# imazen/image-webp

Measured on AMD Instinct MI355X. Metric: 1920x1080 lossy encodes/s (Q75, method 4), higher is better.
Workload: dtype int32; 1 GPU; encode_frame_lossy 1920x1080 RGBA Q75 m4; device_batch=1024, distinct_frames=4, mbs_per_frame=8160, parallelism=frames sharded over 1 GPU(s), steps_pipelined=True, pipeline_lanes=2

## Files before the change

image-webp_amd/csrc/zw_enc_kernels.hip:

```cpp
#include "zw_dev.h"

#include <type_traits>

#include "zw_enc_rows.h"
#include "zw_enc_pairfinal.h"

#define ZW_PH_N 28

#ifdef ZW_NW
#define ZW_NW1 ZW_NW
#define ZW_NW2 ZW_NW
#endif
#ifndef ZW_NW1
#define ZW_NW1 12
#endif
#ifndef ZW_NW2
#define ZW_NW2 12
#endif
#define NW_MAX (ZW_NW1 > ZW_NW2 ? ZW_NW1 : ZW_NW2)
#ifndef ZW_DYN_PRIO
#define ZW_DYN_PRIO 1
#endif
#ifndef ZW_DYN_PRIO1
#define ZW_DYN_PRIO1 2
#endif
#ifndef ZW_P1_LUMA_MAX
#define ZW_P1_LUMA_MAX 3
#endif
#ifndef ZW_CHAIN_PRIO
#define ZW_CHAIN_PRIO 3
#endif
#ifndef ZW_LUMA_PRIO
#define ZW_LUMA_PRIO 0
#endif

template <int PASS> struct PassShape {
    static constexpr int NW = PASS == 1 ? ZW_NW1 : ZW_NW2;
    static constexpr int WG = NW * 64;
};

struct EncArgs {
    const uint8_t *Y, *U, *V;
    const uint8_t* alpha;
    const ZwFrameParams* params;
    const ZwLevelCosts* lcost;
    int8_t* derr;
    ZwMbOut* out;
    uint8_t *ry, *ru, *rv;
    size_t ysz, csz;
    int mbw, mbh, pass;
    int* dbg;
    uint8_t* rows;
    uint32_t* sizes;
    int nframes;
};

struct MbLds {
    uint8_t sy[256], su[64], sv[64];
    uint8_t ws[17 * ZW_BPS];
    uint8_t left_y[20], left_u[12], left_v[12], left_c[12];
    int8_t left_derr[4];
    uint8_t modes[16];
    int16_t lev[25][16];
};

struct WaveLds {
    MbLds mb;
    uint8_t cu[9 * ZW_BPS], cv[9 * ZW_BPS];
    uint32_t uvc[64][8];
    int dc[64];
    int y2d[64];
    int y2cost[4];
    int V[2][40];
    int nzt[4], nzl[4];
    int misc[16];
    uint32_t pst[2][4];
    uint8_t win_y[32], win_u[8], win_v[8], win_c[12];
    int8_t win_d[4];
#ifdef ZW_PHASE_PROF
    unsigned long long ph[ZW_PH_N];
#endif
};


struct Ctx {
    const EncArgs* a;
    const ZwFrameParams* P;
    int method;
    const ZwSegment* S;
    const ZwSegment* Sl;
    const LdsTables* T;
    WaveLds* W;
    MbLds* M;
    uint8_t *top_y, *top_u, *top_v, *top_c;
    int8_t* top_derr;
    const uint8_t *srcY, *srcU, *srcV;
    const uint8_t *sY, *sU, *sV;
    int ys, cs;
    int mbx, mby, lane, seg;
    int f;
    int oy, oc, ocx, od;
};

__device__ void build_luma_border(const Ctx& C, int part = 2)
{
    uint8_t* ws = C.M->ws;
    const int l = C.lane;
    const int mbw = C.a->mbw;
    const bool want = part == 2 || (part == 0 ? (l < 17 || l >= 32) : (l >= 17 && l < 32));
    if (!want) {
    } else if (l < 32) {
        int v;
        if (l == 0) v = C.mby == 0 ? 127 : (C.mbx == 0 ? 129 : C.M->left_y[0]);
        else if (C.mby == 0) v = 127;
        else if (l <= 16) v = C.top_y[C.oy + l - 1];
        else if (C.mbx == mbw - 1) v = C.top_y[C.oy + 15];
        else v = C.top_y[C.oy + l - 1];
        ws[l] = (uint8_t)v;
        if (l >= 17 && l < 21) {
            ws[4 * ZW_BPS + l] = (uint8_t)v;
            ws[8 * ZW_BPS + l] = (uint8_t)v;
            ws[12 * ZW_BPS + l] = (uint8_t)v;
        }
    } else if (l < 48) {
        int i = l - 32;
        ws[(i + 1) * ZW_BPS] = C.mbx == 0 ? 129 : C.M->left_y[1 + i];
    }
    wsync();
}

__device__ void build_chroma_border(const Ctx& C)
{
    const int l = C.lane;
    if (l < 34) {
        const int pl = l >= 17;
        const int i = pl ? l - 17 : l;
// ... 1641 lines not shown
            }
        }
#pragma unroll
        for (int k = 0; k < 8; k++)
            asm volatile("v_writelane_b32 %0, %1, %2" : "+v"(cf[0][0]) : "s"(__builtin_amdgcn_readfirstlane(dcs[k])), "i"(k));
    }
    int dq[2][4];
    int nz = 0;
#pragma unroll
    for (int c = 0; c < 2; c++)
#pragma unroll
        for (int r = 0; r < 4; r++) {
            const bool dcs = c == 0 && r == 0;
            const uint32_t iq = dcs ? (h ? S.uv.iq[1] : S.uv.iq[0]) : S.uv.iq[1];
            const uint32_t bias = dcs ? (h ? S.uv.bias[1] : S.uv.bias[0]) : S.uv.bias[1];
            const int q_ = dcs ? (int)(h ? S.uv.q[1] : S.uv.q[0]) : (int)S.uv.q[1];
            const int lv = quantz(cf[c][r], iq, bias);
            nz |= lv;
            if (act) C.M->lev[17 + b][izz_of(4 * r + 2 * h + c)] = (int16_t)lv;
            dq[c][r] = m24(lv, q_);
        }
    uint32_t r01[2], r32[2];
    idct_recon_pair(dq, p01, p32, h, r01, r32);
    if (act) {
        uint8_t* w = pl ? W->cv : W->cu;
#pragma unroll
        for (int r = 0; r < 2; r++) {
            uint8_t* row = w + (by * 4 + 2 * h + r + 1) * ZW_BPS + 1 + bx * 4;
            row[0] = (uint8_t)(r01[r] & 255u);
            row[1] = (uint8_t)(r01[r] >> 16);
            row[2] = (uint8_t)(r32[r] >> 16);
            row[3] = (uint8_t)(r32[r] & 255u);
        }
    }
    const int nzb = (nz | hx_partner(nz)) != 0;
    int any = 0;
#pragma unroll
    for (int k = 0; k < 8; k++) {
        uv_nz[k] = __builtin_amdgcn_readlane(nzb, k);
        any |= uv_nz[k];
    }
    wsync();
    return any;
}

__device__ void store_luma_borders(const Ctx& C)
{
    const int l = C.lane;
    if (l < 17) C.M->left_y[l] = C.M->ws[l * ZW_BPS + 16];
    else if (l < 33) C.top_y[C.oy + (l - 17)] = C.M->ws[16 * ZW_BPS + (l - 17) + 1];
    if (C.a->ry && l < 64) {
        uint8_t* ry = C.a->ry + (size_t)C.f * C.a->ysz + (size_t)C.mby * 16 * C.ys + C.mbx * 16;
        for (int k = l; k < 256; k += 64) ry[(size_t)(k >> 4) * C.ys + (k & 15)] = C.M->ws[((k >> 4) + 1) * ZW_BPS + 1 + (k & 15)];
    }
    wsync();
}
__device__ void store_chroma_borders(const Ctx& C)
{
    const int l = C.lane;
    WaveLds* W = C.W;
    if (l < 9) {
        C.M->left_u[l] = W->cu[l * ZW_BPS + 8];
        C.M->left_v[l] = W->cv[l * ZW_BPS + 8];
    } else if (l < 17) {
        C.top_u[C.oc + (l - 9)] = W->cu[8 * ZW_BPS + (l - 9) + 1];
        C.top_v[C.oc + (l - 9)] = W->cv[8 * ZW_BPS + (l - 9) + 1];
    }
    if (C.a->ru) {
        uint8_t* ru = C.a->ru + (size_t)C.f * C.a->csz + (size_t)C.mby * 8 * C.cs + C.mbx * 8;
        uint8_t* rv = C.a->rv + (size_t)C.f * C.a->csz + (size_t)C.mby * 8 * C.cs + C.mbx * 8;
        const int k = l;
        ru[(size_t)(k >> 3) * C.cs + (k & 7)] = W->cu[((k >> 3) + 1) * ZW_BPS + 1 + (k & 7)];
        rv[(size_t)(k >> 3) * C.cs + (k & 7)] = W->cv[((k >> 3) + 1) * ZW_BPS + 1 + (k & 7)];
    }
    wsync();
}

__device__ void write_levels(const Ctx& C, int first_blk, int nblk, bool zero)
{
    ZwMbOut* o = C.a->out + (size_t)C.f * C.a->mbw * C.a->mbh + (size_t)C.mby * C.a->mbw + C.mbx;
    uint32_t* dst = (uint32_t*)&o->levels[first_blk][0];
    const uint32_t* srcl = (const uint32_t*)&C.M->lev[first_blk][0];
    for (int k = C.lane; k < nblk * 8; k += 64) dst[k] = zero ? 0u : srcl[k];
}

struct UvQ {
    int pl;
    uint8_t* w;
    const uint8_t* sp;
    uint8_t* top;
    uint8_t* left;
};

DI void uvq_border(const Ctx& C, const UvQ& U)
{
    const int l = C.lane;
    if (l < 17) {
        if (l == 0) U.w[0] = C.mby == 0 ? 127 : (C.mbx == 0 ? 129 : U.left[0]);
        else if (l <= 8) U.w[l] = C.mby == 0 ? 127 : U.top[C.mbx * 8 + l - 1];
        else U.w[(l - 8) * ZW_BPS] = C.mbx == 0 ? 129 : U.left[l - 8];
    }
    wsync();
}

DI int uvq_rcost(const int av[4], int q, const LdsTables* T)
{
    unsigned nz = 0, big = 0;
    int part = 0;
#pragma unroll
    for (int r = 0; r < 4; r++) {
        const int n = 4 * r + q;
        nz |= (unsigned)min(av[r], 1) << n;
        big |= (unsigned)(av[r] >= 2) << n;
        part += T->lfc[min(av[r], 2047)];
    }
    nz = (unsigned)quad_or((int)nz);
    big = (unsigned)quad_or((int)big);
    const int sum = quad_sum(part);
    const int last = 31 - __clz((int)nz);
    const int ctx_t = ((big >> max(last, 0)) & 1u) ? 2 : 1;
    const int tail = (int)T->beob[2][band_of(min(last + 1, 15))][ctx_t] & -(int)(last < 15);
    const int head = (int)T->binit[2][0][0];
    return csel(last < 0, (int)T->beob[2][0][0], head + sum + tail);
}

DI int uvq_pick(const Ctx& C, const UvQ& U, int* xch, int* xflag, int seq)
{
    const ZwSegment& S = *C.S;
    const LdsTables* T = C.T;
    WaveLds* W = C.W;
    const int l = C.lane, m = l >> 4, b = (l >> 2) & 3, q = l & 3, bx = b & 1, by = b >> 1;
    const int above = C.mby != 0, left = C.mbx != 0;
    int dc;
    {
        const int i = l & 15;
        const int v = (int)U.w[csel(i < 8, (i + 1) * ZW_BPS, i - 7)] & -(int)(i < 8 ? left : above);
        const int su = __builtin_amdgcn_readlane(red16(v), 0);
        const int shf = 2 + left + above;
        dc = (above | left) ? (su + (1 << (shf - 1))) >> shf : 128;
    }
    uint32_t p01, p32, s01, s32;
    {
        const int cm = -(int)(m & 1), rm = -(int)(m >= 2);
        const int P = U.w[0];
        const int ro = csel(m == 0, dc, csel(m == 3, -P, 0));
        const uint8_t* tp = U.w + 1 + bx * 4;
        const uint32_t c01 = pack_lo(tp[0] & cm, tp[1] & cm), c32 = pack_lo(tp[3] & cm, tp[2] & cm);
        const int y = by * 4 + q;
        const int rv = (U.w[(y + 1) * ZW_BPS] & rm) + ro;
        const uint32_t rvv = pack_lo(rv, rv);
        p01 = clamp_pk(add_pk(c01, rvv));
        p32 = clamp_pk(add_pk(c32, rvv));
        const uint32_t sw = *(const uint32_t*)(U.sp + y * 8 + bx * 4);
        s01 = __builtin_amdgcn_perm(0u, sw, 0x0c010c00u);
        s32 = __builtin_amdgcn_perm(0u, sw, 0x0c020c03u);
    }
    const uint32_t R01 = sub_pk(s01, p01), R32 = sub_pk(s32, p32);
    int cf[4];
    uvq_fdct(add_pk(R01, R32), sub_pk(R01, R32), q, cf);
    {
        uint32_t* e = W->uvc[l];
        e[0] = pack_lo(cf[0], cf[1]);
        e[1] = pack_lo(cf[2], cf[3]);
        e[2] = p01;
        e[3] = p32;
    }
// ... 501 lines not shown
template <int PASS> DI void luma_issue_prio(const int* progress, int prevw, int mbx, int mby, int mbw)
{
#if ZW_DYN_PRIO > 0
    int slack = mbw;
    if (mby > 0) {
        const int v = __builtin_amdgcn_readfirstlane(
            __hip_atomic_load(&progress[prevw], __ATOMIC_RELAXED, __HIP_MEMORY_SCOPE_WORKGROUP));
        if ((v >> 16) == mby - 1) slack = (v & 0xffff) - mbx - 1;
    }
    constexpr int dp = PASS == 1 ? ZW_DYN_PRIO1 : ZW_DYN_PRIO;
    const int p = slack >= dp * 3 ? 3 : (slack >= dp * 2 ? 2 : (slack >= dp ? 1 : 0));
    set_prio(PASS == 1 ? min(p, ZW_P1_LUMA_MAX) : p);
#endif
}

DI uint32_t mb_luma(Ctx& C, int lm, bool i4reuse, uint32_t i4nz, bool trel)
{
    int ynz[16];
    uint32_t r = (uint32_t)(final_luma(C, lm, trel, ynz, i4reuse ? (int)i4nz : -1) != 0) << 16;
#pragma unroll
    for (int k = 0; k < 16; k++) r |= (uint32_t)(ynz[k] != 0) << k;
    return r;
}
DI uint32_t mb_chroma(Ctx& C, int cm)
{
    int uvnz[8];
    uint32_t r = (uint32_t)(final_chroma(C, cm, C.top_derr + C.od, uvnz) != 0) << 8;
#pragma unroll
    for (int k = 0; k < 8; k++) r |= (uint32_t)(uvnz[k] != 0) << k;
    return r;
}
template <int PASS> DI void mb_finish(Ctx& C, int lm, int cm, uint32_t lres, uint32_t cres, bool chroma_borders)
{
    const EncArgs& a = *C.a;
    const int lane = C.lane, mbw = a.mbw;
    const size_t nmb = (size_t)mbw * a.mbh;
    int ynz[16], uvnz[8];
#pragma unroll
    for (int k = 0; k < 16; k++) ynz[k] = (int)((lres >> k) & 1u);
#pragma unroll
    for (int k = 0; k < 8; k++) uvnz[k] = (int)((cres >> k) & 1u);
    const int lnz = (int)((lres >> 16) & 1u), cnz = (int)((cres >> 8) & 1u);
    ZwMbOut* o = a.out + (size_t)C.f * nmb + (size_t)C.mby * mbw + C.mbx;
    if (PASS == 2) {
        const int skip = !(lnz | cnz);
        if (lane == 0) {
            uint8_t* tc = C.top_c + C.ocx;
            uint8_t* lc = C.M->left_c;
            if (skip) {
                for (int k = 1; k < 9; k++) tc[k] = lc[k] = 0;
                if (lm != 4) tc[0] = lc[0] = 0;
            } else {
                if (lm != 4) {
                    int y2nz = 0;
                    for (int n = 0; n < 16; n++) y2nz |= C.M->lev[16][n] != 0;
                    tc[0] = lc[0] = (uint8_t)y2nz;
                }
                for (int x = 0; x < 4; x++) tc[1 + x] = (uint8_t)ynz[12 + x];
                for (int y = 0; y < 4; y++) lc[1 + y] = (uint8_t)ynz[y * 4 + 3];
                tc[5] = (uint8_t)uvnz[2];
                tc[6] = (uint8_t)uvnz[3];
                lc[5] = (uint8_t)uvnz[1];
                lc[6] = (uint8_t)uvnz[3];
                tc[7] = (uint8_t)uvnz[6];
                tc[8] = (uint8_t)uvnz[7];
                lc[7] = (uint8_t)uvnz[5];
                lc[8] = (uint8_t)uvnz[7];
            }
            o->skip = (uint8_t)skip;
            o->chroma_mode = (uint8_t)cm;
        }
        if (chroma_borders) store_chroma_borders(C);
        write_levels(C, 0, 25, skip);
        if (a.sizes) {
            int e = 0;
            if (lane < 25 && !skip) {
                const uint32_t* lw = (const uint32_t*)C.M->lev[lane];
#pragma unroll
                for (int q = 0; q < 8; q++) {
                    const uint32_t v = lw[q];
                    e = (v >> 16) ? 2 * q + 2 : ((v & 0xffffu) ? 2 * q + 1 : e);
                }
            }
            const int r16 = red16(e);
            const int es = __builtin_amdgcn_readlane(r16, 0) + __builtin_amdgcn_readlane(r16, 16);
            if (lane == 0)
                a.sizes[(size_t)C.f * nmb + (size_t)C.mby * mbw + C.mbx] = (uint32_t)(1 + (lm == 4 ? 8 : 0) + 25 + 2 * es);
        }
    } else {
        write_levels(C, 0, 17, false);
        if (lane == 0) o->skip = 0;
    }
    if (lane == 0) {
        o->luma_mode = (uint8_t)lm;
        o->segment = (uint8_t)C.seg;
    }
    if (lane < 16) o->bpred[lane] = lm == 4 ? C.M->modes[lane] : 0;
    store_luma_borders(C);
}
template <int PASS> DI void mb_store(Ctx& C, int lm, int cm, bool i4reuse, uint32_t i4nz, bool trel)
{
    [[maybe_unused]] const int lane = C.lane;
    PH_START();
    const uint32_t lres = mb_luma(C, lm, i4reuse, i4nz, trel);
    PH_MARK(4);
    const uint32_t cres = PASS == 2 ? mb_chroma(C, cm) : 0u;
    PH_MARK(5);
    mb_finish<PASS>(C, lm, cm, lres, cres, true);
}

template <int PASS> DI void chain_quad(const EncWg& G, Ctx& C)
{
    const EncArgs& a = *G.a;
    const int mbw = a.mbw, mbh = a.mbh, f = G.f, lane = C.lane;
    const size_t nmb = (size_t)mbw * mbh;
    if (lane < 4) C.M->left_derr[lane] = 0;
    const int pl = __builtin_amdgcn_readfirstlane(G.wv);
    UvQ U;
    U.pl = pl;
    U.w = G.W->cu;
    U.sp = C.M->su;
    U.top = pl ? G.top_v : G.top_u;
    U.left = C.M->left_u;
    const uint8_t* const P0 = (pl ? a.V : a.U) + (size_t)f * a.csz;
    const int cs = mbw * 8;
    auto fetch_uv = [&](int mbx, int mby) {
        MbFetch r;
        r.y = lane < 16 ? *(const uint32_t*)(P0 + (size_t)(mby * 8 + (lane >> 1)) * cs + mbx * 8 + (lane & 1) * 4) : 0u;
        r.c = 0;
        r.alpha = a.alpha[(size_t)f * nmb + (size_t)mby * mbw + mbx];
        return r;
    };
    C.ys = mbw * 16;
    C.cs = cs;
    MbFetch nx = fetch_uv(0, 0);
    int seq = 0;
    for (int mby = 0; mby < mbh; mby++) {
        if (lane < 12) C.M->left_u[lane] = 129;
        wsync();
        for (int mbx = 0; mbx < mbw; mbx++) {
            PH_START();
            const int lane = opaque_lane(threadIdx.x & 63);
            C.lane = lane;
            const MbFetch cur = nx;
            if (mbx + 1 < mbw) nx = fetch_uv(mbx + 1, mby);
            else if (mby + 1 < mbh) nx = fetch_uv(0, mby + 1);
            C.mbx = mbx;
            C.mby = mby;
            if (lane < 16) ((uint32_t*)C.M->su)[lane] = cur.y;
            wsync();
            const int seg = __builtin_amdgcn_readfirstlane((int)G.seg_lut[cur.alpha]);
            C.seg = seg;
            C.S = C.Sl + seg;
            uvq_border(C, U);
            const int cm = uvq_pick(C, U, G.xch, G.xflag, ++seq);
            PH_MARK(8);
            uvq_final(C, U, cm, G.top_derr + mbx * 4);
            PH_MARK(9);
            uvq_store_borders(C, U);
            ZwMbOut* o = a.out + (size_t)f * nmb + (size_t)mby * mbw + mbx;
            if (pl == 0 && lane == 0) o->chroma_mode = (uint8_t)cm;
            write_levels(C, 17 + 4 * pl, 4, false);
            wsync();
        }
    }
    for (int i = lane; i < mbw * 2; i += 64) {
        const int j = (i >> 1) * 4 + pl * 2 + (i & 1);
        a.derr[(size_t)f * mbw * 4 + j] = G.top_derr[j];
    }
}

template <int PASS, int FP> DI void chain_one(const EncWg& G, Ctx& C)
{
    const EncArgs& a = *G.a;
    const int mbw = a.mbw, mbh = a.mbh, lane = C.lane;
    const size_t nmb = (size_t)mbw * mbh;
    const int cfr = FP == 2 ? G.wv : 0;
    const bool has_chain = cfr < G.nf;
    const FrameLds F = frame_lds<PASS>(G, cfr);
    ctx_enter(C, F, &G.W->mb, 0, 0);
    if (lane < 4) C.M->left_derr[lane] = 0;
    MbFetch nx = fetch_mb(&a, F.f, lane, 0, 0);
    for (int mby = 0; has_chain && mby < mbh; mby++) {
        if (lane < 12) {
            C.M->left_u[lane] = 129;
            C.M->left_v[lane] = 129;
        }
        wsync();
        for (int mbx = 0; mbx < mbw; mbx++) {
            PH_START();
            const int lane = opaque_lane(threadIdx.x & 63);
            C.lane = lane;
            const MbFetch cur = nx;
            if (mbx + 1 < mbw) nx = fetch_mb(&a, F.f, lane, mbx + 1, mby);
            else if (mby + 1 < mbh) nx = fetch_mb(&a, F.f, lane, 0, mby + 1);
            setup_ctx(C, &a, F.seg_lut, G.W, mbx, mby, cur);
            C.oc = mbx * 8;
            C.ocx = mbx * 12;
            build_chroma_border(C);
            const int cm = pick_uv<PASS>(C);
            PH_MARK(8);
            int uvnz[8];
            final_chroma(C, cm, F.top_derr + mbx * 4, uvnz);
            PH_MARK(9);
            store_chroma_borders(C);
            ZwMbOut* o = a.out + (size_t)F.f * nmb + (size_t)mby * mbw + mbx;
            if (lane == 0) o->chroma_mode = (uint8_t)cm;
            write_levels(C, 17, 8, false);
            wsync();
        }
    }
    for (int i = lane; has_chain && i < mbw * 4; i += 64) a.derr[(size_t)F.f * mbw * 4 + i] = F.top_derr[i];
}

DI void ctx_pair(const Ctx& C, const FrameLds& F0, const FrameLds& F1, MbLds* const Mp[2], int mbx, int mby, int seg0,
                 int seg1, Ctx& CA, Ctx& CB)
{
    CA = CB = C;
    CA.lane = CB.lane = opaque_lane(threadIdx.x & 63);
    ctx_enter(CA, F0, Mp[0], mbx, mby);
    ctx_enter(CB, F1, Mp[1], mbx, mby);
    CA.seg = seg0;
    CB.seg = seg1;
    CA.S = CA.Sl + seg0;
    CB.S = CB.Sl + seg1;
}

template <int PASS, int NW, int NCW> DI void luma_pairs(const EncWg& G, Ctx& C)
{
    const EncArgs& a = *G.a;
    WaveLds* const W = G.W;
    int* const progress = G.progress;
    const int mbw = a.mbw, mbh = a.mbh, lane = C.lane;
    const int nf = __builtin_amdgcn_readfirstlane(G.nf), wv = __builtin_amdgcn_readfirstlane(G.wv);
    const FrameLds F[2] = {frame_lds<PASS>(G, 0), frame_lds<PASS>(G, 1)};
    MbLds* const Mp[2] = {&W->mb, G.M2};
    const int K = F[0].method <= 3 ? 3 : (F[0].method == 4 ? 4 : 10);
    const bool same_k = nf == 1 || (F[1].method == F[0].method && F[1].trel == F[0].trel);
    using RP = typename std::conditional<PASS == 1, PairRowSchedule1<NW, NCW>, RowSchedule<PASS, false, NW, NCW, true>>::type;
    for (int mby = RP::first_row(wv, mbh); mby < mbh; mby = RP::next_row(wv, mby, mbh)) {
#pragma unroll
        for (int fr = 0; fr < 2; fr++) row_start(Mp[fr], lane);
        wsync();
        const int prevw = __builtin_amdgcn_readfirstlane(mby > 0 ? RP::wave_of_row(mby - 1, mbh) : 0);
        auto wait_above = [&](int need) {
            if (mby > 0) wait_row(progress, prevw, (mby - 1) * 65536 + need);
        };
        for (int mbx = 0; mbx < mbw; mbx++) {
            PH_START();
            const int lane = opaque_lane(threadIdx.x & 63);
            C.lane = lane;
            auto enter = [&](int fr) {
                C.lane = opaque_lane(threadIdx.x & 63);
                ctx_enter(C, F[fr], Mp[fr], mbx, mby);
            };
            auto pst = [&](int fr, int k) { return (uint32_t)__builtin_amdgcn_readfirstlane((int)W->pst[fr][k]); };
            auto enter_seg = [&](int fr, uint32_t sm) {
                enter(fr);
                C.seg = (int)(sm >> 8);
                C.S = C.Sl + C.seg;
            };
            wait_above(min(mbx + 1, mbw));
            luma_issue_prio<PASS>(progress, prevw, mbx, mby, mbw);
            PH_MARK(0);
#pragma unroll
            for (int fr = 0; fr < 2; fr++) {
                if (fr >= nf) {
                    if (lane == 0) W->pst[fr][0] = 0;
                    continue;
                }
                enter(fr);
                const MbFetch fm = fetch_mb(&a, C.f, lane, mbx, mby);
                setup_ctx(C, &a, F[fr].seg_lut, W, mbx, mby, fm);
                build_luma_border(C, 0);
                int l_;
                unsigned long long s_;
                pick_i16<PASS>(C, l_, s_);
                const bool n_ = C.method > 1 && (C.method >= 5 || s_ > 211ull * C.S->l_mode || l_ != 0);
                if (lane == 0) {
                    W->pst[fr][0] = (uint32_t)l_ | ((uint32_t)n_ << 4) | ((uint32_t)C.seg << 8);
                    W->pst[fr][1] = (uint32_t)s_;
                    W->pst[fr][2] = (uint32_t)(s_ >> 32);
                    W->pst[fr][3] = 0;
                }
                wsync();
            }
            wsync();
            PH_MARK(1);
            const uint32_t s0 = pst(0, 0), s1 = pst(1, 0);
            const bool n0 = (s0 >> 4) & 1u, n1 = (s1 >> 4) & 1u;
            if (n0 || n1) wait_above(min(mbx + 2, mbw));
// ... 223 lines not shown
template <int PASS, bool ROWS, int FP = 1> DI void encode_body(const EncArgs& a)
{
    using SH = EncShape<PASS, ROWS, FP>;
    extern __shared__ __attribute__((aligned(16))) uint8_t smem[];
    const int lane = threadIdx.x & 63;
    const EncWg G = enc_carve<PASS, ROWS, FP>(a, smem);
    const bool chain_wg = PASS == 1 && (ROWS ? blockIdx.x == 0 : G.wv < SH::NCW);
    enc_fill<PASS, ROWS, FP>(G, chain_wg);

    Ctx C;
    C.a = &a;
    C.W = G.W;
    C.lane = lane;
    ctx_enter(C, frame_lds<PASS>(G, 0), &G.W->mb, 0, 0);
    ph_init(G, lane);

    if (chain_wg) {
        __builtin_amdgcn_s_setprio(ZW_CHAIN_PRIO);
        if constexpr (SH::NCH == 2 && !SH::PAIR) chain_quad<PASS>(G, C);
        else chain_one<PASS, FP>(G, C);
    }
    if (!chain_wg || SH::PAIR) {
        if (PASS == 1) __builtin_amdgcn_s_setprio(ZW_LUMA_PRIO);
        if constexpr (SH::PAIR) luma_pairs<PASS, SH::NW, SH::NCW>(G, C);
        else luma_rows<PASS, ROWS, SH::NW, SH::NCH>(G, C);
    }
    ph_flush<PASS>(G, lane);
}

extern "C" __global__ __launch_bounds__(PassShape<1>::WG) void k_encode_pass1(EncArgs a) { encode_body<1, false>(a); }
extern "C" __global__ __launch_bounds__(PassShape<1>::WG) void k_encode_pass1_fp(EncArgs a) { encode_body<1, false, 2>(a); }
extern "C" __global__ __launch_bounds__(PassShape<2>::WG) void k_encode_pass2(EncArgs a) { encode_body<2, false>(a); }
extern "C" __global__ __launch_bounds__(PassShape<2>::WG) void k_encode_pass2_fp(EncArgs a) { encode_body<2, false, 2>(a); }
extern "C" __global__ __launch_bounds__(64 * RowsShape<1>::NW) void k_encode_rows_pass1(EncArgs a) { encode_body<1, true>(a); }
extern "C" __global__ __launch_bounds__(64) void k_encode_rows_pass2(EncArgs a) { encode_body<2, true>(a); }

static size_t encode_lds_bytes(int mbw, int nw, bool rows, int pass, int fp = 1)
{
    return EncLds(mbw, rows, pass).bytes(nw, fp);
}

static bool encode_fp_for(int pass, int mbw, int nframes)
{
    static const int mode2 = [] { const char* e = getenv("ZW_ENC_FP"); return e && *e ? atoi(e) : -1; }();
    static const int mode1 = [] { const char* e = getenv("ZW_ENC_FP1"); return e && *e ? atoi(e) : mode2; }();
    const int mode = pass == 1 ? mode1 : mode2;
    static const int cus = [] {
        int dev = 0;
        hipDeviceProp_t prop;
        return hipGetDevice(&dev) == hipSuccess && hipGetDeviceProperties(&prop, dev) == hipSuccess &&
                       prop.multiProcessorCount > 0
                   ? prop.multiProcessorCount
                   : 256;
    }();
    if (mode == 0 || nframes < 2) return false;
    if (encode_lds_bytes(mbw, pass == 1 ? PassShape<1>::NW : PassShape<2>::NW, false, pass, 2) > 160 * 1024) return false;
    return mode == 1 || nframes >= 2 * cus;
}
extern "C" int zwk_encode_fp(int pass, int mbw, int nframes) { return encode_fp_for(pass, mbw, nframes) ? 1 : 0; }

extern "C" int zwk_encode_max_mbw(int rows)
{
    int lo = 1, hi = 65536 / 16;
    while (lo < hi) {
        const int mid = (lo + hi + 1) / 2;
        const bool ok = rows ? encode_lds_bytes(mid, RowsShape<1>::NW, true, 1) <= 160 * 1024 &&
                                   encode_lds_bytes(mid, RowsShape<2>::NW, true, 2) <= 160 * 1024
                             : encode_lds_bytes(mid, PassShape<1>::NW, false, 1) <= 160 * 1024 &&
                                   encode_lds_bytes(mid, PassShape<2>::NW, false, 2) <= 160 * 1024;
        if (ok) lo = mid;
        else hi = mid - 1;
    }
    return lo;
}

extern "C" size_t zwk_encode_rows_bytes(int mbw, int mbh, int nframes)
{
    return ZW_ROWS_HDR + (size_t)nframes * RowsLayout(mbw, mbh).frame;
}

extern "C" hipError_t zwk_encode(hipStream_t s, int pass, const uint8_t* Y, const uint8_t* U, const uint8_t* V,
                                 const uint8_t* alpha, const ZwFrameParams* params, const ZwLevelCosts* lcost,
                                 int8_t* derr, ZwMbOut* out, uint8_t* ry, uint8_t* ru, uint8_t* rv, size_t ysz,
                                 size_t csz, int mbw, int mbh, int nframes, int* dbg, uint8_t* rows, uint32_t* sizes)
{
    EncArgs a;
    a.dbg = dbg;
    a.sizes = pass == 2 ? sizes : nullptr;
    a.Y = Y; a.U = U; a.V = V; a.alpha = alpha; a.params = params; a.lcost = lcost; a.derr = derr; a.out = out;
    a.ry = ry; a.ru = ru; a.rv = rv; a.ysz = ysz; a.csz = csz; a.mbw = mbw; a.mbh = mbh; a.pass = pass;
    a.rows = rows;
    a.nframes = nframes;
    static const bool attr_set = []() {
        (void)hipFuncSetAttribute((const void*)k_encode_pass1, hipFuncAttributeMaxDynamicSharedMemorySize, 160 * 1024);
        (void)hipFuncSetAttribute((const void*)k_encode_pass2, hipFuncAttributeMaxDynamicSharedMemorySize, 160 * 1024);
        (void)hipFuncSetAttribute((const void*)k_encode_pass2_fp, hipFuncAttributeMaxDynamicSharedMemorySize, 160 * 1024);
        (void)hipFuncSetAttribute((const void*)k_encode_pass1_fp, hipFuncAttributeMaxDynamicSharedMemorySize, 160 * 1024);
        (void)hipFuncSetAttribute((const void*)k_encode_rows_pass1, hipFuncAttributeMaxDynamicSharedMemorySize, 160 * 1024);
        (void)hipFuncSetAttribute((const void*)k_encode_rows_pass2, hipFuncAttributeMaxDynamicSharedMemorySize, 160 * 1024);
        return true;
    }();
    (void)attr_set;
    if (rows) {
        if (pass == 1) {
            constexpr int nw = RowsShape<1>::NW;
            hipLaunchKernelGGL(k_encode_rows_pass1, dim3(1 + (mbh + nw - 1) / nw, nframes), dim3(64 * nw),
                               encode_lds_bytes(mbw, nw, true, 1), s, a);
        } else {
            hipLaunchKernelGGL(k_encode_rows_pass2, dim3(mbh, nframes), dim3(64), encode_lds_bytes(mbw, 1, true, 2), s,
                               a);
        }
        return hipGetLastError();
    }
    if (encode_fp_for(pass, mbw, nframes)) {
        if (pass == 1)
            hipLaunchKernelGGL(k_encode_pass1_fp, dim3((nframes + 1) / 2), dim3(PassShape<1>::WG),
                               encode_lds_bytes(mbw, PassShape<1>::NW, false, 1, 2), s, a);
        else
            hipLaunchKernelGGL(k_encode_pass2_fp, dim3((nframes + 1) / 2), dim3(PassShape<2>::WG),
                               encode_lds_bytes(mbw, PassShape<2>::NW, false, 2, 2), s, a);
        return hipGetLastError();
    }
    const size_t lds = encode_lds_bytes(mbw, pass == 1 ? PassShape<1>::NW : PassShape<2>::NW, false, pass);
    if (pass == 1) hipLaunchKernelGGL(k_encode_pass1, dim3(nframes), dim3(PassShape<1>::WG), lds, s, a);
    else hipLaunchKernelGGL(k_encode_pass2, dim3(nframes), dim3(PassShape<2>::WG), lds, s, a);
    return hipGetLastError();
}
```

image-webp_amd/csrc/zw_host.cpp:

```cpp
#include <hip/hip_runtime.h>
#include <immintrin.h>

#include <algorithm>
#include <chrono>
#include <atomic>
#include <sys/resource.h>
#include <sys/syscall.h>
#include <unistd.h>
#include <time.h>
#include <condition_variable>
#include <mutex>
#include <new>
#include <cstdio>
#include <cstdlib>
#include <cstring>
#include <deque>
#include <memory>
#include <thread>
#include <vector>

#include "../../include/zwebp.h"
#include "zw_common.h"
#include "zw_host_emit.h"
#include "zw_host_internal.h"
#include "zw_ingest.h"
#include "zw_progress.h"

extern "C" {
hipError_t zwk_rgb2yuv(hipStream_t s, const uint8_t* img, int w, int h, int bpp, int mbw, int mbh, uint8_t* Y,
                       uint8_t* U, uint8_t* V, size_t img_stride, size_t ysz, size_t csz, int nframes);
hipError_t zwk_rgb2yuv_dev(hipStream_t s, const void* data, int layout, int dtype, int channels, size_t frame_stride,
                           size_t plane_stride, size_t row_stride, const float* scale, const float* bias, int w, int h,
                           int mbw, int mbh, uint8_t* Y, uint8_t* U, uint8_t* V, size_t ysz, size_t csz, int nframes);
hipError_t zwk_analysis(hipStream_t s, const uint8_t* Y, const uint8_t* U, const uint8_t* V, int mbw, int mbh,
                        size_t ysz, size_t csz, uint8_t* alpha, uint32_t* histo, int nframes);
hipError_t zwk_segments(hipStream_t s, uint32_t* histo, const ZwFrameParams* tmpl, ZwFrameParams* params,
                        int nframes);
hipError_t zwk_stats(hipStream_t s, const ZwMbOut* mbs, int mbw, int mbh, void* scratch, void* out, int nframes);
size_t zw_stats_scratch_bytes(int nmb, int nframes);
hipError_t zwk_pack(hipStream_t s, const ZwMbOut* mbs, int nmb, int nframes, uint8_t* eobs, uint32_t* sizes,
                     unsigned long long* counter, unsigned long long* frame_info, uint8_t* out, int sizes_ready);
hipError_t zwk_fdct_quant(hipStream_t s, const void* src, const void* pred, size_t n, const ZwMatrix* m, int first,
                          void* levels, void* recon, int cus);
hipError_t zwk_xform_mb(hipStream_t s, const uint8_t* Y, const uint8_t* U, const uint8_t* V, int src_bpp, int w,
                        int h, size_t img_stride, const uint8_t* recs, const void* segs, int mbw, int mbh, int nframes,
                        int16_t* levels, uint8_t* RY, uint8_t* RU, uint8_t* RV, uint32_t* queue, int qp,
                        uint32_t* qerr, int variant);
size_t zwk_xform_mb_seg_bytes(void);
size_t zwk_xform_mb_queue_bytes(int mbw, int mbh, int nframes);
void zwk_xform_mb_pack_segs(const ZwMatrix* m, int n, void* out);
hipError_t zwk_quant_blocks(hipStream_t s, const int* coeffs, const uint8_t* ctx0s, const ZwLevelCosts* lcost,
                            const uint8_t* probs, const void* args, int* levels, int* dq);
hipError_t zwk_encode(hipStream_t s, int pass, const uint8_t* Y, const uint8_t* U, const uint8_t* V,
                      const uint8_t* alpha, const ZwFrameParams* params, const ZwLevelCosts* lcost, int8_t* derr,
                      ZwMbOut* out, uint8_t* ry, uint8_t* ru, uint8_t* rv, size_t ysz, size_t csz, int mbw, int mbh,
                      int nframes, int* dbg, uint8_t* rows, uint32_t* sizes = nullptr);
size_t zwk_encode_rows_bytes(int mbw, int mbh, int nframes);
int zwk_encode_max_mbw(int rows);
int zwk_encode_fp(int pass, int mbw, int nframes);
}

extern "C" const char* zw_strerror(int code)
{
    switch (code) {
    case ZW_OK: return "ok";
    case ZW_EINVALID_DIMENSIONS: return "invalid dimensions";
    case ZW_EINVALID_BUFFER_SIZE: return "invalid buffer size";
    case ZW_EINVAL: return "invalid argument";
    case ZW_EDEVICE: return "device error";
    case ZW_EUNSUPPORTED: return "unsupported";
    case ZW_ENOMEM: return "out of memory";
    case ZW_EVP8_MAGIC: return "invalid VP8 magic";
    case ZW_ECOLORSPACE: return "invalid VP8 color space";
    case ZW_ELUMA_MODE: return "invalid luma prediction mode";
    case ZW_EINTRA_MODE: return "invalid intra prediction mode";
    case ZW_ECHROMA_MODE: return "invalid chroma prediction mode";
    case ZW_EBITSTREAM: return "bitstream error";
    case ZW_EUNSUPPORTED_FEATURE: return "unsupported feature";
    case ZW_ENOT_ENOUGH_INIT_DATA: return "not enough VP8 init data";
    case ZW_ECHUNK_HEADER: return "invalid chunk header";
    case ZW_EWEBP_SIGNATURE: return "invalid WEBP signature";
    case ZW_ECHUNK_MISSING: return "an expected chunk was missing";
    case ZW_EINCONSISTENT_SIZES: return "inconsistent image sizes";
    case ZW_EIMAGE_TOO_LARGE: return "image too large";
    case ZW_EALPHA_PREPROCESSING: return "invalid alpha preprocessing";
    case ZW_ECOMPRESSION_METHOD: return "invalid compression method";
    case ZW_EHUFFMAN: return "invalid lossless Huffman code";
    case ZW_ETRANSFORM: return "invalid lossless transform";
    case ZW_ECOLOR_CACHE_BITS: return "invalid color cache bits";
    case ZW_ELOSSLESS_SIGNATURE: return "invalid lossless signature";
    case ZW_EVERSION_NUMBER: return "invalid lossless version number";
    default: return "unknown error";
    }
}

static std::atomic<int> g_ctx_alive{0};
bool zw_ctx_any_alive() { return g_ctx_alive.load(std::memory_order_acquire) > 0; }

extern "C" int zw_ctx_create(int device, zw_ctx** out)
{
    if (!out) return ZW_EINVAL;
    *out = nullptr;
    int n = 0;
    if (hipGetDeviceCount(&n) != hipSuccess || n <= 0 || device < 0 || device >= n) return ZW_EDEVICE;
    HIPOK(hipSetDevice(device));
    zw_ctx* c = new zw_ctx();
    c->device = device;
    g_ctx_alive.fetch_add(1, std::memory_order_acq_rel);
    *out = c;
    return ZW_OK;
}

struct AgentFind {
    uint32_t bdf, domain;
    hsa_agent_t gpu{}, cpu{};
    bool gpu_ok = false, cpu_ok = false;
};
static hsa_status_t find_agents_cb(hsa_agent_t a, void* data)
{
    AgentFind* F = (AgentFind*)data;
    hsa_device_type_t t;
    if (hsa_agent_get_info(a, HSA_AGENT_INFO_DEVICE, &t) != HSA_STATUS_SUCCESS) return HSA_STATUS_SUCCESS;
    if (t == HSA_DEVICE_TYPE_CPU && !F->cpu_ok) {
        F->cpu = a;
        F->cpu_ok = true;
    } else if (t == HSA_DEVICE_TYPE_GPU) {
        uint32_t bdf = 0, dom = 0;
        (void)hsa_agent_get_info(a, (hsa_agent_info_t)HSA_AMD_AGENT_INFO_BDFID, &bdf);
        (void)hsa_agent_get_info(a, (hsa_agent_info_t)HSA_AMD_AGENT_INFO_DOMAIN, &dom);
        if (bdf == F->bdf && dom == F->domain) {
            F->gpu = a;
            F->gpu_ok = true;
        }
    }
    return HSA_STATUS_SUCCESS;
}

static int sdma_probe_locked(zw_ctx* c)
{
// ... 276 lines not shown
    size_t n = 0;
    bool alloc(size_t count)
    {
        free();
        if (hipHostMalloc((void**)&p, count * sizeof(T) + 64, hipHostMallocDefault) != hipSuccess) {
            p = nullptr;
            return false;
        }
        n = count;
        memset((void*)p, 0, count * sizeof(T));
        return true;
    }
    void free()
    {
        pinned_free(p);
        p = nullptr;
        n = 0;
    }
    T* data() { return p; }
    T& operator[](size_t i) { return p[i]; }
    const T& operator[](size_t i) const { return p[i]; }
    size_t size() const { return n; }
    ~Pinned() { free(); }
};

struct FetchBuf {
    uint8_t* pack = nullptr;
    size_t cap = 0;
    Pinned<unsigned long long> finfo;
    Pinned<unsigned long long> total;
    void release()
    {
        pinned_free(pack);
        pack = nullptr;
        cap = 0;
    }
};

enum LaneEvent { EV_YUV_BEGIN, EV_YUV_END, EV_P1_BEGIN, EV_P1_END, EV_P2_BEGIN, EV_P2_END, EV_STATS_QUEUED, EV_COUNT };
enum KernelMs { KMS_RGB2YUV, KMS_ANALYSIS, KMS_PASS1, KMS_PASS2, KMS_COUNT };
enum HostMs { HMS_FETCH, HMS_STATS, HMS_FETCH2, HMS_EMIT, HMS_COUNT };
enum { PIPE_MS_HOST = KMS_COUNT, PIPE_MS_EMIT_CPU = KMS_COUNT + HMS_COUNT, PIPE_MS_COUNT };

struct PipeLane {
    int f0 = 0, n = 0;
    int chunk = 0;
    hipStream_t stream = nullptr;
    std::vector<hipEvent_t> cev;
    static int pass_slot(int c, int pass) { return 2 * c + pass - 1; }
    hipEvent_t pass_done(int c, int pass) const { return cev[pass_slot(c, pass)]; }
    hipEvent_t ev[EV_COUNT] = {};
    unsigned long long* d_ctr = nullptr;
    uint8_t* d_rows = nullptr;
    FetchBuf fb[3];
    Pinned<ZwStatsOut> h_stats;
    float kms[KMS_COUNT] = {0, 0, 0, 0};
    double hms[HMS_COUNT] = {0, 0, 0, 0};
    double emit_cpu_ms = 0;
    bool pair2 = false;
    int p2_frames = 0;
    bool pair1 = false;
    int p1_frames = 0;
    int rc = 0;
    std::vector<hipStream_t> ustreams;
    std::vector<hipEvent_t> uev[2], rev[2];
    std::vector<uint8_t*> ustage;
    std::vector<hsa_signal_t> usig;
};

struct zw_pipe {
    zw_ctx* ctx;
    int n, w, h, color, bpp, quality, method, mbw, mbh, nmb, qi, filter;
    size_t img_stride, ysz, csz;
    uint8_t *d_img = nullptr, *d_Y = nullptr, *d_U = nullptr, *d_V = nullptr;
    uint8_t *d_ry = nullptr, *d_ru = nullptr, *d_rv = nullptr, *d_alpha = nullptr;
    uint32_t* d_histo = nullptr;
    ZwFrameParams *d_tmpl = nullptr, *d_params = nullptr;
    ZwLevelCosts* d_lcost = nullptr;
    int8_t* d_derr = nullptr;
    ZwMbOut *d_out1 = nullptr, *d_out2 = nullptr;
    int* d_dbg = nullptr;
    ZwStatsOut* d_stats = nullptr;
    void* d_stats_tmp = nullptr;
    bool host_stats = false;
    uint8_t* d_eobs = nullptr;
    uint32_t* d_sizes = nullptr;
    unsigned long long *d_finfo = nullptr, *d_finfo2 = nullptr;
    uint8_t *d_pack = nullptr, *d_pack2 = nullptr;
    size_t pack_stride = 0;
    Pinned<ZwFrameParams> h_params;
    Pinned<ZwLevelCosts> h_lcost;
    std::vector<uint8_t> h_have_upd;
    std::vector<uint8_t> h_upd;
    int out_par = 0;
    std::vector<std::vector<uint8_t>> bitstreams;
    bool container = false;
    std::vector<const uint8_t*> host_frames;
    int nparts = 1;
    std::vector<PipeLane> lanes;
    std::vector<Progress> p1_stats;
    float kms[PIPE_MS_COUNT] = {0, 0, 0, 0, 0, 0, 0, 0, 0};
    bool trace = false;
    double trace_t0 = 0;
    std::mutex ews_mu;
    std::vector<std::unique_ptr<zwh::EmitWs>> ews;
    bool broken = false;
    uint8_t* d_img2 = nullptr;
    const uint8_t* const* host_src = nullptr;
    bool up_pack = false;
    uint8_t* img_buf(int parity) const { return parity ? d_img2 : d_img; }
    zw_device_images dev_in = {};
};

static void pipe_free(zw_pipe* p)
{
    if (!p) return;
    if (p->ctx && p->ctx->poisoned.load(std::memory_order_acquire)) p->d_img = p->d_img2 = nullptr;
    void* ptrs[] = {p->d_img, p->d_img2, p->d_Y, p->d_U, p->d_V, p->d_ry, p->d_ru, p->d_rv, p->d_alpha, p->d_histo,
                    p->d_tmpl, p->d_params, p->d_lcost, p->d_derr, p->d_out1, p->d_out2, p->d_dbg,
                    p->d_eobs, p->d_sizes, p->d_finfo, p->d_pack, p->d_finfo2, p->d_pack2, p->d_stats, p->d_stats_tmp};
    for (void* q : ptrs)
        if (q) (void)hipFree(q);
    for (PipeLane& L : p->lanes) {
        if (L.d_ctr) (void)hipFree(L.d_ctr);
        if (L.d_rows) (void)hipFree(L.d_rows);
        for (FetchBuf& b : L.fb) b.release();
        for (hipEvent_t e : L.ev)
            if (e) (void)hipEventDestroy(e);
        for (hipEvent_t e : L.cev)
            if (e) (void)hipEventDestroy(e);
        if (L.stream) (void)hipStreamDestroy(L.stream);
        for (hipStream_t u : L.ustreams) (void)hipStreamDestroy(u);
        for (uint8_t* b : L.ustage) pinned_free(b);
        if (!g_dma_poisoned.load())
            for (hsa_signal_t sg : L.usig) (void)hsa_signal_destroy(sg);
        for (int k = 0; k < 2; k++) {
            for (hipEvent_t e : L.uev[k])
                if (e) (void)hipEventDestroy(e);
            for (hipEvent_t e : L.rev[k])
                if (e) (void)hipEventDestroy(e);
        }
    }
    delete p;
}

static int pipe_lanes_for(int n, int device, int mbw)
{
    const char* e = getenv("ZW_PIPE_LANES");
    int g;
    if (e && *e) {
        g = atoi(e);
    } else {
        const int cus = device_cus(device);
        const bool fp = zwk_encode_fp(2, mbw, 2 * cus) != 0;
        g = n >= (fp ? 4 : 2) * cus ? 2 : 1;
    }
    if (g < 1) g = 1;
    if (g > 16) g = 16;
    while (g > 1 && n / g < 8) g--;
    return g;
}
static int pipe_chunk_for(int lane_frames, int device)
{
    const char* e = getenv("ZW_PIPE_CHUNK");
    int c = e ? atoi(e) : 0;
    if (c < 1) c = device_cus(device);
    return c > lane_frames ? lane_frames : c;
}
static bool pipe_rows_for(int chunk, int mbw, int mbh, int device)
{
    static const int batch_max_mbw = zwk_encode_max_mbw(0);
    if (mbw > batch_max_mbw) return true;
    const char* e = getenv("ZW_ENC_ROWS");
    if (e && *e) return atoi(e) != 0;
    return (long long)chunk * (mbh + 1) <= 12LL * device_cus(device);
}

extern "C" int zw_pipe_create(zw_ctx* ctx, int n, uint32_t width, uint32_t height, int color, uint8_t quality,
                              uint8_t method, zw_pipe** out)
{
    if (!ctx || !out || n <= 0) return ZW_EINVAL;
    *out = nullptr;
    if (!encode_dims_ok(width, height)) return ZW_EINVALID_DIMENSIONS;
    if (color < 0 || color > 3) return ZW_EINVAL;
    if (quality > 100) return ZW_EINVAL;
    HIPOK(hipSetDevice(ctx->device));
    zw_pipe* p = new zw_pipe();
    p->ctx = ctx;
    p->n = n;
    p->w = (int)width;
    p->h = (int)height;
    p->color = color;
    static const int bpp_of[4] = {1, 2, 3, 4};
    p->bpp = bpp_of[color];
    p->quality = quality;
    p->method = method > 6 ? 6 : method;
    p->mbw = (p->w + 15) / 16;
    p->mbh = (p->h + 15) / 16;
    p->nmb = p->mbw * p->mbh;
    p->img_stride = (size_t)p->w * p->h * p->bpp;
    p->ysz = (size_t)p->mbw * 16 * p->mbh * 16;
    p->csz = (size_t)p->mbw * 8 * p->mbh * 8;
    p->qi = zwh::quality_to_qi(quality);
    p->filter = zwh::filter_level_for(p->qi);
    p->pack_stride = (size_t)p->nmb * (1 + 8 + 25 + 800);
    const size_t N = (size_t)n;
    bool ok = hipMalloc(&p->d_img, N * p->img_stride + 64) == hipSuccess &&
              hipMalloc(&p->d_Y, N * p->ysz) == hipSuccess && hipMalloc(&p->d_U, N * p->csz) == hipSuccess &&
              hipMalloc(&p->d_V, N * p->csz) == hipSuccess && hipMalloc(&p->d_ry, N * p->ysz) == hipSuccess &&
              hipMalloc(&p->d_ru, N * p->csz) == hipSuccess && hipMalloc(&p->d_rv, N * p->csz) == hipSuccess &&
              hipMalloc(&p->d_alpha, N * p->nmb) == hipSuccess &&
              hipMalloc(&p->d_histo, N * 256 * sizeof(uint32_t)) == hipSuccess &&
              hipMalloc(&p->d_tmpl, sizeof(ZwFrameParams)) == hipSuccess &&
              hipMalloc(&p->d_params, N * sizeof(ZwFrameParams)) == hipSuccess &&
              hipMalloc(&p->d_lcost, N * sizeof(ZwLevelCosts)) == hipSuccess &&
              hipMalloc(&p->d_derr, N * p->mbw * 4) == hipSuccess &&
              hipMalloc(&p->d_out1, N * p->nmb * sizeof(ZwMbOut)) == hipSuccess &&
              hipMalloc(&p->d_out2, N * p->nmb * sizeof(ZwMbOut)) == hipSuccess &&
              hipMalloc(&p->d_eobs, N * p->nmb * 25) == hipSuccess &&
              hipMalloc(&p->d_sizes, N * p->nmb * sizeof(uint32_t)) == hipSuccess &&
              hipMalloc(&p->d_finfo, N * 2 * sizeof(unsigned long long)) == hipSuccess &&
              hipMalloc(&p->d_pack, N * p->pack_stride) == hipSuccess &&
              hipMalloc(&p->d_finfo2, N * 2 * sizeof(unsigned long long)) == hipSuccess &&
              hipMalloc(&p->d_pack2, N * p->pack_stride) == hipSuccess;
    ok = ok && hipMemset(p->d_histo, 0, N * 256 * sizeof(uint32_t)) == hipSuccess;
    p->host_stats = getenv("ZW_HOST_STATS") != nullptr;
    ok = ok && (p->host_stats || (hipMalloc(&p->d_stats, N * sizeof(ZwStatsOut)) == hipSuccess &&
                                  hipMalloc(&p->d_stats_tmp, zw_stats_scratch_bytes(p->nmb, n)) == hipSuccess));
    const int G = pipe_lanes_for(n, ctx->device, p->mbw);
    p->lanes.resize(G);
    for (int g = 0; ok && g < G; g++) {
        PipeLane& L = p->lanes[g];
        L.f0 = (int)((long long)n * g / G);
        L.n = (int)((long long)n * (g + 1) / G) - L.f0;
        L.chunk = pipe_chunk_for(L.n, ctx->device);
        for (FetchBuf& b : L.fb) ok = ok && b.finfo.alloc(2 * (size_t)L.chunk) && b.total.alloc(1);
        ok = ok && (p->host_stats || L.h_stats.alloc((size_t)L.n));
        const int nch = (L.n + L.chunk - 1) / L.chunk;
        L.cev.assign(2 * (size_t)nch, nullptr);
        ok = ok && hipStreamCreateWithFlags(&L.stream, hipStreamNonBlocking) == hipSuccess &&
             hipMalloc(&L.d_ctr, 2 * (size_t)nch * ZW_PACK_CTR_WORDS * sizeof(unsigned long long)) == hipSuccess &&
             hipMemset(L.d_ctr, 0, 2 * (size_t)nch * ZW_PACK_CTR_WORDS * sizeof(unsigned long long)) == hipSuccess;
        if (ok && pipe_rows_for(L.chunk, p->mbw, p->mbh, ctx->device)) {
            const size_t rb = zwk_encode_rows_bytes(p->mbw, p->mbh, L.chunk);
            ok = hipMalloc(&L.d_rows, rb) == hipSuccess && hipMemset(L.d_rows, 0, rb) == hipSuccess;
            if (ok && getenv("ZW_ENC_FORCE_ERROR")) ok = hipMemset(L.d_rows, 1, 1) == hipSuccess;
        }
        L.pair2 = ok && !L.d_rows && nch >= 2 && zwk_encode_fp(2, p->mbw, 2 * L.chunk);
        L.pair1 = ok && !L.d_rows && nch >= 2 && zwk_encode_fp(1, p->mbw, 2 * L.chunk);
        for (int i = 0; ok && i < EV_COUNT; i++) ok = hipEventCreate(&L.ev[i]) == hipSuccess;
        for (size_t i = 0; ok && i < L.cev.size(); i++)
            ok = hipEventCreateWithFlags(&L.cev[i], hipEventDisableTiming) == hipSuccess;
    }
    if (!ok) {
        pipe_free(p);
        return ZW_ENOMEM;
    }
    if (!p->h_params.alloc(2 * N) || !p->h_lcost.alloc(N)) {
        pipe_free(p);
        return ZW_ENOMEM;
    }
    p->h_have_upd.assign(2 * N, 0);
    p->h_upd.assign(2 * N * 4 * 8 * 3 * 11, 0);
    p->bitstreams.resize(N);
    ZwFrameParams t;
    memset(&t, 0, sizeof t);
    t.width = p->w;
    t.height = p->h;
    t.mbw = p->mbw;
    t.mbh = p->mbh;
    t.method = p->method;
    t.do_trellis = p->method >= 4;
    t.base_qi = p->qi;
    t.filter_level = p->filter;
    t.skip_prob = 200;
    memcpy(t.probs, zwh::COEFF_PROBS, sizeof t.probs);
    if (hipMemcpy(p->d_tmpl, &t, sizeof t, hipMemcpyHostToDevice) != hipSuccess) {
        pipe_free(p);
        return ZW_EDEVICE;
    }
    *out = p;
    return ZW_OK;
}

extern "C" void zw_pipe_destroy(zw_pipe* p)
{
    if (p) (void)hipSetDevice(p->ctx->device);
    pipe_free(p);
}

extern "C" void* zw_pipe_input_device_ptr(zw_pipe* p) { return p ? p->d_img : nullptr; }

extern "C" int zw_pipe_set_container(zw_pipe* p, int enable, const uint8_t* const* host_frames)
{
    if (!p) return ZW_EINVAL;
    if (!enable) {
        p->container = false;
        p->host_frames.clear();
        return ZW_OK;
    }
    const bool has_alpha = p->color == ZW_COLOR_LA8 || p->color == ZW_COLOR_RGBA8;
    if (has_alpha && p->dev_in.data) return ZW_EINVAL;
    if (has_alpha) {
        if (p->w > 16384 || p->h > 16384) return ZW_EINVALID_DIMENSIONS;
        if (!host_frames) return ZW_EINVAL;
        for (int i = 0; i < p->n; i++)
            if (!host_frames[i]) return ZW_EINVAL;
        p->host_frames.assign(host_frames, host_frames + p->n);
    }
    p->container = true;
    return ZW_OK;
// ... 12 lines not shown
        in->capacity < need)
        return ZW_EINVAL;
    const size_t es = (size_t)ing_elsize(in->dtype);
    if (!ing_madd(0, in->capacity, es, &bytes) || ((uintptr_t)in->data & (es - 1))) return ZW_EINVAL;
    HIPOK(hipSetDevice(ctx->device));
    hipPointerAttribute_t at;
    memset(&at, 0, sizeof at);
    if (hipPointerGetAttributes(&at, in->data) != hipSuccess) {
        (void)hipGetLastError();
        return ZW_EINVAL;
    }
    if (at.type != hipMemoryTypeDevice || at.device != ctx->device) return ZW_EINVAL;
    return ZW_OK;
}

extern "C" int zw_pipe_set_input_device(zw_pipe* p, const zw_device_images* in)
{
    if (!p) return ZW_EINVAL;
    if (!in) {
        p->dev_in = zw_device_images{};
        return ZW_OK;
    }
    if (const int r = check_device_input(p->ctx, in, p->n, (uint32_t)p->w, (uint32_t)p->h)) return r;
    if (!((p->color == ZW_COLOR_RGB8 && in->channels == 3) || (p->color == ZW_COLOR_RGBA8 && in->channels == 4)))
        return ZW_EINVAL;
    if (p->container && in->channels == 4) return ZW_EINVAL;
    p->dev_in = *in;
    return ZW_OK;
}

extern "C" int zw_pipe_set_token_partitions(zw_pipe* p, int nparts)
{
    if (!p || (nparts != 1 && nparts != 2 && nparts != 4 && nparts != 8)) return ZW_EINVAL;
    p->nparts = nparts;
    return ZW_OK;
}

extern "C" int zw_pipe_upload(zw_pipe* p, int frame, const uint8_t* data, size_t len)
{
    if (!p || frame < 0 || frame >= p->n || !data) return ZW_EINVAL;
    if (len != p->img_stride) return ZW_EINVALID_BUFFER_SIZE;
    HIPOK(hipMemcpy(p->d_img + (size_t)frame * p->img_stride, data, len, hipMemcpyHostToDevice));
    return ZW_OK;
}

static double now_ms()
{
    return std::chrono::duration<double, std::milli>(std::chrono::steady_clock::now().time_since_epoch()).count();
}
static long long thread_cpu_ns()
{
    timespec ts;
    clock_gettime(CLOCK_THREAD_CPUTIME_ID, &ts);
    return (long long)ts.tv_sec * 1000000000LL + ts.tv_nsec;
}

static hipError_t rows_reset(zw_pipe* p, PipeLane& L, int n)
{
    if (!L.d_rows) return hipSuccess;
    const size_t hdr = zwk_encode_rows_bytes(p->mbw, p->mbh, 0);
    return hipMemsetAsync(L.d_rows + hdr, 0, zwk_encode_rows_bytes(p->mbw, p->mbh, n) - hdr, L.stream);
}
static int rows_check(zw_pipe* p, PipeLane& L)
{
    if (!L.d_rows) return ZW_OK;
    int err = 0;
    HIPOK(hipMemcpy(&err, L.d_rows, sizeof err, hipMemcpyDeviceToHost));
    return err ? ZW_EDEVICE : ZW_OK;
}

static int chunk_pass1_encode(zw_pipe* p, PipeLane& L, int fa, int na, bool timed, bool write_recon = false)
{
    hipStream_t s = L.stream;
    const size_t F = (size_t)fa;
    if (timed) {
        HIPOK(hipEventRecord(L.ev[EV_P1_BEGIN], s));
        L.p1_frames = na;
    }
    HIPOK(rows_reset(p, L, na));
    HIPOK(zwk_encode(s, 1, p->d_Y + F * p->ysz, p->d_U + F * p->csz, p->d_V + F * p->csz, p->d_alpha + F * p->nmb,
                     p->d_params + F, nullptr, p->d_derr + F * p->mbw * 4, p->d_out1 + F * p->nmb,
                     write_recon ? p->d_ry + F * p->ysz : nullptr, write_recon ? p->d_ru + F * p->csz : nullptr,
                     write_recon ? p->d_rv + F * p->csz : nullptr, p->ysz, p->csz, p->mbw, p->mbh, na, nullptr,
                     L.d_rows));
    if (timed) HIPOK(hipEventRecord(L.ev[EV_P1_END], s));
    return ZW_OK;
}

static int chunk_prepass(zw_pipe* p, PipeLane& L, int fa, int na, bool timed, int parity, hipEvent_t uploaded,
                         hipEvent_t read)
{
    hipStream_t s = L.stream;
    const size_t F = (size_t)fa;
    const int n = na;
    if (uploaded) HIPOK(hipStreamWaitEvent(s, uploaded, 0));
    if (timed) HIPOK(hipEventRecord(L.ev[EV_YUV_BEGIN], s));
    const bool packed = uploaded && p->up_pack;
    if (const zw_device_images& D = p->dev_in; D.data) {
        const uint8_t* src = (const uint8_t*)D.data + F * D.frame_stride * (size_t)ing_elsize(D.dtype);
        HIPOK(zwk_rgb2yuv_dev(s, src, D.layout, D.dtype, D.channels, D.frame_stride, D.plane_stride, D.row_stride,
                              D.scale, D.bias, p->w, p->h, p->mbw, p->mbh, p->d_Y + F * p->ysz, p->d_U + F * p->csz,
                              p->d_V + F * p->csz, p->ysz, p->csz, n));
    } else {
        HIPOK(zwk_rgb2yuv(s, p->img_buf(parity) + F * p->img_stride, p->w, p->h, packed ? 3 : p->bpp, p->mbw, p->mbh,
                          p->d_Y + F * p->ysz, p->d_U + F * p->csz, p->d_V + F * p->csz, p->img_stride, p->ysz,
                          p->csz, n));
    }
    if (read) HIPOK(hipEventRecord(read, s));
    if (timed) HIPOK(hipEventRecord(L.ev[EV_YUV_END], s));
    HIPOK(zwk_analysis(s, p->d_Y + F * p->ysz, p->d_U + F * p->csz, p->d_V + F * p->csz, p->mbw, p->mbh, p->ysz,
                       p->csz, p->d_alpha + F * p->nmb, p->d_histo + F * 256, n));
    HIPOK(zwk_segments(s, p->d_histo + F * 256, p->d_tmpl, p->d_params + F, n));
    return ZW_OK;
}

static bool pass2_sizes(const zw_pipe* p) { return p->d_sizes != nullptr; }

static int chunk_pack(zw_pipe* p, PipeLane& L, int fa, int na, const ZwMbOut* d_out, int slot)
{
    const size_t F = (size_t)fa;
    const bool p2 = slot & 1;
    HIPOK(zwk_pack(L.stream, d_out + F * p->nmb, p->nmb, na, p->d_eobs + F * p->nmb * 25, p->d_sizes + F * p->nmb,
                   L.d_ctr + ZW_PACK_CTR_WORDS * slot, (p2 ? p->d_finfo2 : p->d_finfo) + 2 * F,
                   (p2 ? p->d_pack2 : p->d_pack) + F * p->pack_stride, p2 && pass2_sizes(p)));
    return ZW_OK;
}

static int chunk_fetch(zw_pipe* p, PipeLane& L, FetchBuf& B, int fa, int na, int slot, hipEvent_t ready)
{
    const size_t F = (size_t)fa;
    HIPOK(hipEventSynchronize(ready));
    int r = ctx_d2h(p->ctx, B.total.data(), L.d_ctr + ZW_PACK_CTR_WORDS * slot + 2, sizeof(unsigned long long));
    const bool p2 = slot & 1;
    if (!r)
        r = ctx_d2h(p->ctx, B.finfo.data(), (p2 ? p->d_finfo2 : p->d_finfo) + 2 * F,
                    2 * (size_t)na * sizeof(unsigned long long));
    if (r) return r;
    const unsigned long long total = B.total[0];
    if (total > B.cap) {
        B.release();
        const size_t cap = (size_t)(total * 1.25) + 4096;
        if (hipHostMalloc((void**)&B.pack, cap, hipHostMallocDefault) != hipSuccess) return ZW_ENOMEM;
        B.cap = cap;
    }
    return ctx_d2h(p->ctx, B.pack, (p2 ? p->d_pack2 : p->d_pack) + F * p->pack_stride, total);
}

static int chunk_fetch_stats(zw_pipe* p, PipeLane& L, int fa, int na, hipEvent_t ready)
{
    HIPOK(hipEventSynchronize(ready));
    return ctx_d2h(p->ctx, L.h_stats.data() + (fa - L.f0), p->d_stats + fa, (size_t)na * sizeof(ZwStatsOut));
}

static inline size_t hidx(const zw_pipe* p, int par, size_t f) { return (size_t)par * p->n + f; }

static int chunk_stats(zw_pipe* p, PipeLane& L, int fa, int na, int par)
{
    hipStream_t s = L.stream;
    const size_t F = (size_t)fa, n = (size_t)na;
    ZwFrameParams* hp = p->h_params.data() + hidx(p, par, F);
    {
        const int r = ctx_d2h(p->ctx, hp, p->d_params + F, n * sizeof(ZwFrameParams));
        if (r) return r;
    }
    parallel_for(na, [&](int i) {
        const size_t f = F + i, hf = hidx(p, par, f);
        zwh::Stats st;
        int sp;
        if (p->host_stats) {
            sp = zwh::replay_stats(st, L.fb[0].pack + L.fb[0].finfo[2 * i], p->mbw, p->mbh);
        } else {
            const ZwStatsOut& so = L.h_stats[f - L.f0];
            memcpy(st.s, so.s, sizeof st.s);
            sp = zwh::skip_prob(so.total_mbs, so.nonzero_mbs);
        }
        uint8_t* upd = p->h_upd.data() + hf * 4 * 8 * 3 * 11;
        bool have = zwh::updated_probs(st, (uint8_t(*)[8][3][11])upd);
        p->h_have_upd[hf] = have;
        ZwFrameParams& P = p->h_params[hf];
        P.skip_prob = sp;
        memcpy(P.probs, upd, sizeof P.probs);
        zwh::level_costs(p->h_lcost[f], (const uint8_t(*)[8][3][11])upd);
    });
    HIPOK(hipMemcpyAsync(p->d_params + F, hp, n * sizeof(ZwFrameParams), hipMemcpyHostToDevice, s));
    HIPOK(hipMemcpyAsync(p->d_lcost + F, p->h_lcost.data() + F, n * sizeof(ZwLevelCosts), hipMemcpyHostToDevice, s));
    return ZW_OK;
}

static int chunk_pass2(zw_pipe* p, PipeLane& L, int fa, int na, bool timed)
{
    hipStream_t s = L.stream;
    const size_t F = (size_t)fa;
    if (timed) {
        HIPOK(hipEventRecord(L.ev[EV_P2_BEGIN], s));
        L.p2_frames = na;
    }
    HIPOK(rows_reset(p, L, na));
    HIPOK(zwk_encode(s, 2, p->d_Y + F * p->ysz, p->d_U + F * p->csz, p->d_V + F * p->csz, p->d_alpha + F * p->nmb,
                     p->d_params + F, p->d_lcost + F, p->d_derr + F * p->mbw * 4, p->d_out2 + F * p->nmb,
                     p->d_ry + F * p->ysz, p->d_ru + F * p->csz, p->d_rv + F * p->csz, p->ysz, p->csz, p->mbw, p->mbh,
                     na, p->d_dbg ? p->d_dbg + F * p->nmb * 16 * 34 : nullptr, L.d_rows,
                     pass2_sizes(p) ? p->d_sizes + F * p->nmb : nullptr));
    if (timed) HIPOK(hipEventRecord(L.ev[EV_P2_END], s));
    return ZW_OK;
}

static void dump_emit_input(zw_pipe* p, const uint8_t* rec, size_t bytes, size_t hf)
{
    static const char* path = getenv("ZW_DUMP_EMIT");
    static std::atomic<int> done{0};
    if (!path || done.exchange(1)) return;
    FILE* fp = fopen(path, "wb");
    if (!fp) return;
    const uint32_t hdr[4] = {0x4d45575au, (uint32_t)sizeof(ZwFrameParams), (uint32_t)p->w, (uint32_t)p->h};
    const uint8_t have = p->h_have_upd[hf];
    const unsigned long long n = bytes;
    bool ok = fwrite(hdr, sizeof hdr, 1, fp) == 1 && fwrite(&p->h_params[hf], sizeof(ZwFrameParams), 1, fp) == 1 &&
              fwrite(&have, 1, 1, fp) == 1 && fwrite(p->h_upd.data() + hf * 4 * 8 * 3 * 11, 4 * 8 * 3 * 11, 1, fp) == 1 &&
              fwrite(&n, sizeof n, 1, fp) == 1 && fwrite(rec, 1, bytes, fp) == bytes;
    (void)ok;
    fclose(fp);
}

struct EmitWsLease {
    zw_pipe* p;
    std::atomic<long long>& to;
    const long long c0 = thread_cpu_ns();
    std::unique_ptr<zwh::EmitWs> ws;
    EmitWsLease(zw_pipe* p_, std::atomic<long long>& to_) : p(p_), to(to_)
    {
        {
            std::lock_guard<std::mutex> lk(p->ews_mu);
            if (!p->ews.empty()) {
                ws = std::move(p->ews.back());
                p->ews.pop_back();
            }
        }
        if (!ws) ws.reset(new (std::nothrow) zwh::EmitWs);
    }
    ~EmitWsLease()
    {
        if (!ws) return;
        {
            std::lock_guard<std::mutex> lk(p->ews_mu);
            p->ews.push_back(std::move(ws));
        }
        to.fetch_add(thread_cpu_ns() - c0, std::memory_order_relaxed);
    }
};

static int emit_task(zw_pipe* p, const FetchBuf& B, int fa, int par, int i0, int K, zwh::EmitWs* ws)
{
    const size_t F = (size_t)fa;
    const bool has_alpha = p->color == ZW_COLOR_LA8 || p->color == ZW_COLOR_RGBA8;
    std::vector<uint8_t>* vp8 = ws->out;
    std::vector<uint8_t>& alph = ws->alph;
    std::vector<uint8_t>* outs[zwh::EmitWs::kMax];
    for (int k = 0; k < K; k++) {
        const size_t f = F + i0 + k;
        outs[k] = p->container ? &vp8[k] : &p->bitstreams[f];
        outs[k]->clear();
    }
    const ZwFrameParams* Pk[zwh::EmitWs::kMax];
    const uint8_t* rk[zwh::EmitWs::kMax];
    bool hk[zwh::EmitWs::kMax];
    const uint8_t(*uk[zwh::EmitWs::kMax])[8][3][11];
    for (int k = 0; k < K; k++) {
        const size_t hf = hidx(p, par, F + i0 + k);
        Pk[k] = &p->h_params[hf];
        rk[k] = B.pack + B.finfo[2 * (i0 + k)];
        hk[k] = p->h_have_upd[hf] != 0;
        uk[k] = (const uint8_t(*)[8][3][11])(p->h_upd.data() + hf * 4 * 8 * 3 * 11);
    }
    try {
        zwh::emit_frames(outs, Pk, rk, K, p->nparts, p->w, p->h, hk, uk, ws);
    } catch (const std::bad_alloc&) {
        return ZW_ENOMEM;
    }
    if (!p->container) return ZW_OK;
    for (int k = 0; k < K; k++) {
        const size_t f = F + i0 + k;
        std::vector<uint8_t>& out = p->bitstreams[f];
        alph.clear();
        out.clear();
        if (has_alpha) {
// ... 69 lines not shown
        : p(p_), L(L_), emit(emit_), nb(nb_), nch((L_.n + L_.chunk - 1) / L_.chunk), host(p_->host_src != nullptr),
          G((int)p_->lanes.size()), lane_id((int)(&L_ - p_->lanes.data())), p1_order(G > 1 && emit_),
          uploaded(host ? L_.ustreams.size() : 0)
    {
    }
    ~LaneRun()
    {
        join_emitter();
        join_uploaders();
        if (p1_order) p->p1_stats[lane_id].stop();
    }

    int first(int c) const { return L.f0 + c * L.chunk; }
    int count(int c) const { return std::min(L.chunk, L.n - c * L.chunk); }
    template <class F>
    int for_launch_groups(bool paired, F fn) const
    {
        for (int c = 0; c < nch; c++) {
            const int c1 = (paired && (c & 1) == 0 && c + 1 < nch) ? c + 1 : c;
            if (const int r = fn(LaunchGroup{c, c1, first(c), first(c1) + count(c1) - first(c)})) return r;
            c = c1;
        }
        return ZW_OK;
    }
    int join_emitter()
    {
        if (em.joinable()) em.join();
        return emit_rc;
    }
    void join_uploaders()
    {
        if (up.empty()) return;
        if (p1_count < (long long)nb * nch) p1_queued.stop();
        for (auto& t : up) t.join();
        up.clear();
    }

    int p1_order_wait(int b)
    {
        if (!p1_order) return ZW_OK;
        const int prev = (lane_id + G - 1) % G;
        const long long need = lane_id == 0 ? b : b + 1;
        if (need <= 0 || !p->p1_stats[prev].wait_for(need)) return ZW_OK;
        HIPOK(hipStreamWaitEvent(L.stream, p->lanes[prev].ev[EV_STATS_QUEUED], 0));
        return ZW_OK;
    }
    int wait_uploaded(int b, int k)
    {
        for (Progress& u : uploaded)
            if (!u.wait_for((long long)b * nch + k + 1)) return ZW_EDEVICE;
        for (size_t u = 1; u < L.ustreams.size(); u++)
            HIPOK(hipStreamWaitEvent(L.stream, L.uev[b & 1][u * nch + k], 0));
        return ZW_OK;
    }
    int launch_pass1(int b, const LaunchGroup& g)
    {
        if (g.c0 == 0)
            if (const int r = p1_order_wait(b)) return r;
        return chunk_pass1_encode(p, L, g.fa, g.na, g.c0 == 0);
    }
    int queue_pass1_group(int b, const LaunchGroup& g)
    {
        const bool paired = g.c1 != g.c0;
        int r = ZW_OK;
        for (int k = g.c0; k <= g.c1 && !r; k++) {
            if (host && (r = wait_uploaded(b, k))) return r;
            r = chunk_prepass(p, L, first(k), count(k), k == 0, host ? (b & 1) : 0, host ? L.uev[b & 1][k] : nullptr,
                              host ? L.rev[b & 1][k] : nullptr);
            if (!r && !paired) r = launch_pass1(b, g);
            if (host && r) p1_queued.stop();
            if (host && !r) {
                p1_count++;
                p1_queued.advance();
            }
        }
        if (!r && paired) r = launch_pass1(b, g);
        for (int k = g.c0; k <= g.c1 && !r; k++) {
            if (p->host_stats) {
                r = chunk_pack(p, L, first(k), count(k), p->d_out1, PipeLane::pass_slot(k, 1));
            } else {
                const size_t F = (size_t)first(k);
                HIPOK(zwk_stats(L.stream, p->d_out1 + F * p->nmb, p->mbw, p->mbh,
                                (uint8_t*)p->d_stats_tmp + zw_stats_scratch_bytes(p->nmb, (int)F), p->d_stats + F,
                                count(k)));
            }
            if (!r) HIPOK(hipEventRecord(L.pass_done(k, 1), L.stream));
        }
        return r;
    }
    int queue_pass1(int b)
    {
        if (const int r = for_launch_groups(L.pair1, [&](const LaunchGroup& g) { return queue_pass1_group(b, g); }))
            return r;
        if (p1_order) {
            HIPOK(hipEventRecord(L.ev[EV_STATS_QUEUED], L.stream));
            p->p1_stats[lane_id].advance();
        }
        return ZW_OK;
    }
    int stats_and_pass2_group(int b, const LaunchGroup& g)
    {
        int r;
        for (int k = g.c0; k <= g.c1; k++) {
            const double t0 = now_ms();
            r = p->host_stats ? chunk_fetch(p, L, L.fb[0], first(k), count(k), PipeLane::pass_slot(k, 1),
                                            L.pass_done(k, 1))
                              : chunk_fetch_stats(p, L, first(k), count(k), L.pass_done(k, 1));
            if (r) return r;
            const double t1 = now_ms();
            if ((r = chunk_stats(p, L, first(k), count(k), b & 1))) return r;
            ms[HMS_STATS] += now_ms() - t1;
            ms[HMS_FETCH] += t1 - t0;
            if (p->trace)
                fprintf(stderr, "  lane %d batch %d chunk %d: p1 fetched %.1f stats done %.1f\n", L.f0, b, k,
                        t1 - p->trace_t0, now_ms() - p->trace_t0);
            if (emit && b > 0 && !fetched.wait_for((long long)(b - 1) * nch + k + 1)) {
                const int re = join_emitter();
                return re ? re : ZW_EDEVICE;
            }
        }
        r = chunk_pass2(p, L, g.fa, g.na, g.c0 == 0);
        for (int k = g.c0; k <= g.c1 && !r; k++) {
            if (emit) r = chunk_pack(p, L, first(k), count(k), p->d_out2, PipeLane::pass_slot(k, 2));
            if (!r && hipEventRecord(L.pass_done(k, 2), L.stream) != hipSuccess) r = ZW_EDEVICE;
        }
        return r;
    }
    int stats_and_pass2(int b)
    {
        return for_launch_groups(L.pair2, [&](const LaunchGroup& g) { return stats_and_pass2_group(b, g); });
    }
    int run()
    {
        for (int u = 0; u < (int)uploaded.size(); u++) up.emplace_back([this, u] { upload_chunks(u); });
        int r = queue_pass1(0);
        for (int b = 0; b < nb && !r; b++) {
            r = stats_and_pass2(b);
            if (!r && b + 1 < nb) r = queue_pass1(b + 1);
            if (!r && emit && !(r = join_emitter())) em = std::thread([this, b] { emit_thread(b); });
        }
        if (r) return r;
        if ((r = join_emitter())) return r;
        join_uploaders();
        if (up_rc.load()) return up_rc.load();
        p->out_par = (nb - 1) & 1;
        HIPOK(hipStreamSynchronize(L.stream));
        if ((r = rows_check(p, L))) return r;
        for (int i = 0; i < HMS_COUNT; i++) L.hms[i] = ms[i] / nb;
        L.emit_cpu_ms = 1e-6 * (double)emit_cpu.load() / nb;
        lane_times(L);
        return ZW_OK;
    }

    int upload_chunk_dma(int u, int b, int c)
    {
        const int U = (int)L.ustreams.size();
        uint8_t* dst = p->img_buf(b & 1) + (size_t)first(c) * p->img_stride;
        int r = ZW_OK;
        if (b >= 2 && hipEventSynchronize(L.rev[b & 1][c]) != hipSuccess) r = ZW_EDEVICE;
        bool busy[2] = {false, false};
        int k = 0;
        for (int i = u; i < count(c) && !r; i += U, k++) {
            const int sl = k & 1;
            if (busy[sl] && (r = sdma_wait(p->ctx, L.usig[2 * u + sl]))) break;
            const uint8_t* src = p->host_src[(size_t)b * p->n + first(c) + i];
            size_t bytes = p->img_stride;
            if (p->up_pack) {
// ... 223 lines not shown
                L.usig.push_back(sg);
            }
        }
        for (int k = 0; k < 2; k++) {
            while ((int)L.uev[k].size() < U * nch) {
                hipEvent_t a = nullptr;
                HIPOK(hipEventCreateWithFlags(&a, hipEventDisableTiming));
                L.uev[k].push_back(a);
            }
            while ((int)L.rev[k].size() < nch) {
                hipEvent_t a = nullptr;
                HIPOK(hipEventCreateWithFlags(&a, hipEventDisableTiming));
                L.rev[k].push_back(a);
            }
        }
    }
    {
        const char* pe = getenv("ZW_UPLOAD_PACK");
        p->up_pack = p->bpp == 4 && !p->lanes.empty() && !p->lanes[0].ustage.empty() && !(pe && atoi(pe) == 0);
    }
    p->host_src = frames;
    const int r = pipe_encode(p, nb);
    p->host_src = nullptr;
    p->up_pack = false;
    return r;
}

extern "C" int zw_pipe_encode_repeat(zw_pipe* p, int n) { return pipe_encode(p, n); }

extern "C" int zw_pipe_launch_frames(zw_pipe* p) { return p && !p->lanes.empty() ? p->lanes[0].chunk : 0; }

extern "C" int zw_pipe_lanes(zw_pipe* p) { return p ? (int)p->lanes.size() : 0; }

extern "C" int zw_pipe_kernel_times(zw_pipe* p, float* ms, int n)
{
    if (!p || !ms) return ZW_EINVAL;
    for (int i = 0; i < n && i < PIPE_MS_COUNT; i++) ms[i] = p->kms[i];
    return ZW_OK;
}

extern "C" int zw_pipe_output(zw_pipe* p, int frame, zw_bytes* out)
{
    if (!p || !out || frame < 0 || frame >= p->n) return ZW_EINVAL;
    const std::vector<uint8_t>& b = p->bitstreams[frame];
    out->data = (uint8_t*)malloc(b.size() ? b.size() : 1);
    if (!out->data) return ZW_ENOMEM;
    memcpy(out->data, b.data(), b.size());
    out->len = b.size();
    return ZW_OK;
}

extern "C" int zw_pipe_read_planes(zw_pipe* p, int frame, int which, uint8_t* y, uint8_t* u, uint8_t* v)
{
    if (!p || frame < 0 || frame >= p->n) return ZW_EINVAL;
    HIPOK(hipSetDevice(p->ctx->device));
    uint8_t* Y = which ? p->d_ry : p->d_Y;
    uint8_t* U = which ? p->d_ru : p->d_U;
    uint8_t* V = which ? p->d_rv : p->d_V;
    if (y) HIPOK(hipMemcpy(y, Y + (size_t)frame * p->ysz, p->ysz, hipMemcpyDeviceToHost));
    if (u) HIPOK(hipMemcpy(u, U + (size_t)frame * p->csz, p->csz, hipMemcpyDeviceToHost));
    if (v) HIPOK(hipMemcpy(v, V + (size_t)frame * p->csz, p->csz, hipMemcpyDeviceToHost));
    return ZW_OK;
}

extern "C" int zw_pipe_read_mbinfo(zw_pipe* p, int frame, int pass, uint8_t* modes, int16_t* levels)
{
    if (!p || frame < 0 || frame >= p->n) return ZW_EINVAL;
    HIPOK(hipSetDevice(p->ctx->device));
    std::vector<ZwMbOut> tmp(p->nmb);
    HIPOK(hipMemcpy(tmp.data(), (pass == 1 ? p->d_out1 : p->d_out2) + (size_t)frame * p->nmb,
                    p->nmb * sizeof(ZwMbOut), hipMemcpyDeviceToHost));
    for (int i = 0; i < p->nmb; i++) {
        if (modes) {
            uint8_t* m = modes + (size_t)i * 20;
            m[0] = tmp[i].luma_mode;
            m[1] = tmp[i].chroma_mode;
            m[2] = tmp[i].skip;
            m[3] = tmp[i].segment;
            memcpy(m + 4, tmp[i].bpred, 16);
        }
        if (levels) memcpy(levels + (size_t)i * 400, tmp[i].levels, 800);
    }
    return ZW_OK;
}

extern "C" int zw_pipe_read_probs(zw_pipe* p, int frame, uint8_t* probs, int* skip_prob)
{
    if (!p || frame < 0 || frame >= p->n) return ZW_EINVAL;
    const ZwFrameParams& P = p->h_params[hidx(p, p->out_par, (size_t)frame)];
    if (probs) memcpy(probs, P.probs, sizeof P.probs);
    if (skip_prob) *skip_prob = P.skip_prob;
    return ZW_OK;
}

extern "C" int zw_pipe_read_segments(zw_pipe* p, int frame, int32_t* seg_qi)
{
    if (!p || frame < 0 || frame >= p->n || !seg_qi) return ZW_EINVAL;
    const ZwFrameParams& P = p->h_params[hidx(p, p->out_par, (size_t)frame)];
    for (int i = 0; i < 4; i++) seg_qi[i] = P.seg[i].quant_index;
    return ZW_OK;
}

extern "C" int zw_pipe_enable_debug(zw_pipe* p)
{
    if (!p) return ZW_EINVAL;
    if (p->d_dbg) return ZW_OK;
    HIPOK(hipSetDevice(p->ctx->device));
    const size_t b = (size_t)p->n * p->nmb * 16 * 34 * sizeof(int);
    if (hipMalloc(&p->d_dbg, b) != hipSuccess) return ZW_ENOMEM;
    HIPOK(hipMemset(p->d_dbg, 0, b));
    return ZW_OK;
}

extern "C" int zw_pipe_read_debug(zw_pipe* p, int frame, int32_t* out)
{
    if (!p || !p->d_dbg || frame < 0 || frame >= p->n || !out) return ZW_EINVAL;
    HIPOK(hipSetDevice(p->ctx->device));
    const size_t b = (size_t)p->nmb * 16 * 34 * sizeof(int);
    HIPOK(hipMemcpy(out, (uint8_t*)p->d_dbg + (size_t)frame * b, b, hipMemcpyDeviceToHost));
    return ZW_OK;
}

extern "C" int zw_pipe_read_alpha(zw_pipe* p, int frame, uint8_t* alpha)
{
    if (!p || frame < 0 || frame >= p->n || !alpha) return ZW_EINVAL;
    HIPOK(hipSetDevice(p->ctx->device));
    HIPOK(hipMemcpy(alpha, p->d_alpha + (size_t)frame * p->nmb, p->nmb, hipMemcpyDeviceToHost));
    return ZW_OK;
}

static int check_encode_args(const uint8_t* data, size_t len, uint32_t width, uint32_t height, int color,
                             uint8_t quality)
{
    if (!encode_dims_ok(width, height)) return ZW_EINVALID_DIMENSIONS;
    if (color < 0 || color > 3) return ZW_EINVAL;
    static const int bpp_of[4] = {1, 2, 3, 4};
    if ((uint64_t)width * height * bpp_of[color] != len || !data) return ZW_EINVALID_BUFFER_SIZE;
    if (quality > 100) return ZW_EINVAL;
    return ZW_OK;
}

extern "C" int zw_encode_batch(zw_ctx* ctx, int n, const zw_image* imgs, uint8_t quality, uint8_t method,
                               zw_bytes* outs)
{
    return zw_encode_batch_ex(ctx, n, imgs, quality, method, 1, outs);
}

extern "C" int zw_encode_batch_ex(zw_ctx* ctx, int n, const zw_image* imgs, uint8_t quality, uint8_t method,
                                  int token_partitions, zw_bytes* outs)
{
    if (!ctx || n <= 0 || !imgs || !outs) return ZW_EINVAL;
    if (token_partitions != 1 && token_partitions != 2 && token_partitions != 4 && token_partitions != 8)
        return ZW_EINVAL;
    for (int i = 0; i < n; i++) {
        outs[i].data = nullptr;
        outs[i].len = 0;
        int r = check_encode_args(imgs[i].data, imgs[i].len, imgs[i].width, imgs[i].height, imgs[i].color, quality);
        if (r) return r;
        if (imgs[i].width != imgs[0].width || imgs[i].height != imgs[0].height || imgs[i].color != imgs[0].color)
            return ZW_EINVAL;
    }
    zw_pipe* p = nullptr;
    int r;
    const int key[5] = {(int)imgs[0].width, (int)imgs[0].height, imgs[0].color, quality, method};
    const bool one = n == 1;
    if (one) {
// ... 647 lines not shown
```

image-webp_amd/csrc/zw_pack_kernels.hip:

```cpp
#include "zw_dev.h"

#ifndef PK_WAVES
#define PK_WAVES 4
#endif

__device__ __forceinline__ int pk_mb_size(int luma, int eobsum) { return 1 + (luma == 4 ? 8 : 0) + 25 + 2 * eobsum; }

__device__ __forceinline__ int pk_word_eob(uint32_t v, int j)
{
    const int n0 = 2 * (j & 7);
    return (v >> 16) ? n0 + 2 : ((v & 0xffffu) ? n0 + 1 : 0);
}
__device__ __forceinline__ int max8(int e)
{
    e = max(e, __builtin_amdgcn_mov_dpp(e, 0xB1, 0xf, 0xf, false));
    e = max(e, __builtin_amdgcn_mov_dpp(e, 0x4E, 0xf, 0xf, false));
    e = max(e, __builtin_amdgcn_mov_dpp(e, 0x141, 0xf, 0xf, false));
    return e;
}

extern "C" __global__ __launch_bounds__(64 * PK_WAVES) void k_pack_size(const ZwMbOut* __restrict__ mbs, int nmb,
                                                                      int nframes, uint8_t* __restrict__ eobs,
                                                                      uint32_t* __restrict__ sizes)
{
    const size_t mb = (size_t)blockIdx.x * PK_WAVES + (threadIdx.x >> 6);
    const int lane = threadIdx.x & 63;
    if (mb >= (size_t)nmb * nframes) return;
    const ZwMbOut& M = mbs[mb];
    const uint32_t* W = (const uint32_t*)&M.levels[0][0];
    uint32_t w[4];
#pragma unroll
    for (int r = 0; r < 4; r++) w[r] = lane + 64 * r < 200 ? W[lane + 64 * r] : 0u;
    const int skip = M.skip;
    int s = 0;
#pragma unroll
    for (int r = 0; r < 4; r++) {
        const int j = lane + 64 * r;
        const int eob = skip ? 0 : max8(pk_word_eob(w[r], j));
        if ((j & 7) == 0 && j < 200) {
            eobs[mb * 25 + (j >> 3)] = (uint8_t)eob;
            s += eob;
        }
    }
#pragma unroll
    for (int o = 32; o >= 1; o >>= 1) s += __shfl_xor(s, o);
    if (lane == 0) sizes[mb] = (uint32_t)pk_mb_size(M.luma_mode, s);
}

extern "C" __global__ __launch_bounds__(1024) void k_pack_scan(uint32_t* __restrict__ sizes, int nmb,
                                                              unsigned long long* __restrict__ counter,
                                                              unsigned long long* __restrict__ frame_info)
{
    __shared__ uint32_t part[1024];
    __shared__ unsigned long long base;
    const int f = blockIdx.x, t = threadIdx.x;
    uint32_t* S = sizes + (size_t)f * nmb;
    const int per = (nmb + 1023) / 1024;
    const int b0 = t * per, b1 = min(b0 + per, nmb);
    uint32_t acc = 0;
    for (int i = b0; i < b1; i++) acc += S[i];
    part[t] = acc;
    __syncthreads();
    for (int o = 1; o < 1024; o <<= 1) {
        const uint32_t v = t >= o ? part[t - o] : 0;
        __syncthreads();
        part[t] += v;
        __syncthreads();
    }
    uint32_t run = part[t] - acc;
    for (int i = b0; i < b1; i++) {
        const uint32_t v = S[i];
        S[i] = run;
        run += v;
    }
    if (t == 1023) {
        const unsigned long long tot = part[1023];
        base = atomicAdd(counter, tot);
        frame_info[2 * f] = base;
        frame_info[2 * f + 1] = tot;
        __threadfence();
        if (atomicAdd(counter + 1, 1ull) == (unsigned long long)gridDim.x - 1) {
            __threadfence();
            const unsigned long long all = atomicAdd(counter, 0ull);
            counter[2] = all;
            atomicExch(counter, 0ull);
            atomicExch(counter + 1, 0ull);
        }
    }
}

extern "C" __global__ __launch_bounds__(64 * PK_WAVES) void k_pack_write(
    const ZwMbOut* __restrict__ mbs, int nmb, int nframes, const uint8_t* __restrict__ eobs,
    const uint32_t* __restrict__ offs, const unsigned long long* __restrict__ frame_info, uint8_t* __restrict__ out)
{
    const size_t mb = (size_t)blockIdx.x * PK_WAVES + (threadIdx.x >> 6);
    const int lane = threadIdx.x & 63;
    if (mb >= (size_t)nmb * nframes) return;
    const int f = (int)(mb / nmb);
    const ZwMbOut& M = mbs[mb];
    const uint32_t* W = (const uint32_t*)&M.levels[0][0];
    uint32_t w[4];
#pragma unroll
    for (int r = 0; r < 4; r++) w[r] = lane + 64 * r < 200 ? W[lane + 64 * r] : 0u;
    const uint32_t hw = *(const uint32_t*)&M;
    const uint32_t bp = lane < 8 ? *(const uint16_t*)&M.bpred[2 * lane] : 0u;
    uint8_t* o = out + frame_info[2 * f] + offs[mb];
    const int luma = (int)(hw & 255u), chroma = (int)((hw >> 8) & 255u), skip = (int)((hw >> 16) & 255u),
              seg = (int)(hw >> 24);
    const int hdr = 1 + (luma == 4 ? 8 : 0);
    int eb4[4];
#pragma unroll
    for (int r = 0; r < 4; r++) eb4[r] = skip ? 0 : max8(pk_word_eob(w[r], lane + 64 * r));
    int eob = 0;
#pragma unroll
    for (int r = 0; r < 4; r++) {
        const int v = __shfl(eb4[r], 8 * (lane & 7));
        eob = (lane >> 3) == r ? v : eob;
    }
    eob = lane < 25 ? eob : 0;
    if (lane == 0) o[0] = (uint8_t)(luma | (skip << 3) | (seg << 4) | (chroma << 6));
    if (luma == 4 && lane < 8) o[1 + lane] = (uint8_t)((bp & 15u) | (((bp >> 8) & 15u) << 4));
    if (lane < 25) o[hdr + lane] = (uint8_t)eob;
    int pre = eob;
#pragma unroll
    for (int d = 1; d < 32; d <<= 1) {
        const int v = __shfl_up(pre, d);
        if (lane >= d) pre += v;
    }
    pre -= eob;
    int16_t* lv = (int16_t*)(o + hdr + 25);
#pragma unroll
    for (int r = 0; r < 4; r++) {
        const int j = lane + 64 * r;
        const int b = min(j >> 3, 24), n0 = 2 * (j & 7);
        const int eb = eb4[r], st = __shfl(pre, b);
        if (j < 200 && n0 < eb) {
            const uint32_t v = w[r];
            lv[st + n0] = (int16_t)(v & 0xffffu);
            if (n0 + 1 < eb) lv[st + n0 + 1] = (int16_t)(v >> 16);
        }
    }
}

extern "C" hipError_t zwk_pack(hipStream_t s, const ZwMbOut* mbs, int nmb, int nframes, uint8_t* eobs, uint32_t* sizes,
                               unsigned long long* counter, unsigned long long* frame_info, uint8_t* out,
                               int sizes_ready)
{
    const size_t total = (size_t)nmb * nframes;
    const unsigned grid = (unsigned)((total + PK_WAVES - 1) / PK_WAVES);
    if (!sizes_ready)
        hipLaunchKernelGGL(k_pack_size, dim3(grid), dim3(64 * PK_WAVES), 0, s, mbs, nmb, nframes, eobs, sizes);
    hipLaunchKernelGGL(k_pack_scan, dim3(nframes), dim3(1024), 0, s, sizes, nmb, counter, frame_info);
    hipLaunchKernelGGL(k_pack_write, dim3(grid), dim3(64 * PK_WAVES), 0, s, mbs, nmb, nframes, eobs, sizes, frame_info,
                       out);
    return hipGetLastError();
}
```

image-webp_amd/csrc/zw_stats_kernels.hip:

```cpp
#include "zw_dev.h"

#define ZS_WG 1024
#ifndef ZS_STRIPE
#define ZS_STRIPE 128
#endif
#ifndef ZS_COPIES
#define ZS_COPIES 4
#endif
static_assert((ZS_STRIPE * 25 + ZS_COPIES - 1) / ZS_COPIES * 9 < 65536, "a packed 16:16 copy must not carry");
#ifndef ZS_HWG
#define ZS_HWG 512
#endif
#define ZS_NCTR (4 * 8 * 3 * 11)

typedef ZwStatsOut StatsOut;

__device__ __forceinline__ int zs_band(int n) { return n >= 16 ? 0 : (int)((0x7666666665463210ull >> (4 * n)) & 15); }

__device__ __forceinline__ int zs_eob(const int16_t* lv)
{
    const uint32_t* w = (const uint32_t*)lv;
    int e = 0;
#pragma unroll
    for (int q = 0; q < 8; q++) {
// ... 38 lines not shown
                    fn(C(band, ctx, 4), 0);
                } else {
                    fn(C(band, ctx, 4), 1);
                    fn(C(band, ctx, 5), v == 4);
                }
            } else if (v <= 10) {
                fn(C(band, ctx, 3), 1);
                fn(C(band, ctx, 6), 0);
                fn(C(band, ctx, 7), v > 6);
            } else {
                fn(C(band, ctx, 3), 1);
                fn(C(band, ctx, 6), 1);
                if (v < 35) {
                    fn(C(band, ctx, 8), 0);
                    fn(C(band, ctx, 9), v >= 19);
                } else {
                    fn(C(band, ctx, 8), 1);
                    fn(C(band, ctx, 10), v >= 67);
                }
            }
            ctx = 2;
        }
    }
    if (n < 16) fn(C(zs_band(n), ctx, 0), 0);
}

#define ZS_I4 (1u << 25)
#define ZS_SKIP (1u << 26)

template <class FL>
__device__ __forceinline__ int zs_ctx_f(FL&& flag, int mb, int mbx, int mby, int mbw, int b)
{
    auto nz = [&](int m, int bb) -> int { return (int)((flag(m) >> bb) & 1u); };
    int l = 0, t = 0;
    if (b < 16) {
        const int bx = b & 3, by = b >> 2;
        l = bx > 0 ? nz(mb, b - 1) : (mbx > 0 ? nz(mb - 1, b + 3) : 0);
        t = by > 0 ? nz(mb, b - 4) : (mby > 0 ? nz(mb - mbw, b + 12) : 0);
    } else if (b == 16) {
        for (int x = mbx - 1; x >= 0; x--)
            if (!(flag(mb - (mbx - x)) & ZS_I4)) {
                l = nz(mb - (mbx - x), 16);
                break;
            }
        for (int y = mby - 1; y >= 0; y--)
            if (!(flag(mb - (mby - y) * mbw) & ZS_I4)) {
                t = nz(mb - (mby - y) * mbw, 16);
                break;
            }
    } else {
        const int bb = (b - 17) & 3, bx = bb & 1, by = bb >> 1;
        l = bx > 0 ? nz(mb, b - 1) : (mbx > 0 ? nz(mb - 1, b + 1) : 0);
        t = by > 0 ? nz(mb, b - 2) : (mby > 0 ? nz(mb - mbw, b + 2) : 0);
    }
    return min(l + t, 2);
}
__device__ __forceinline__ int zs_ctx(const uint32_t* fl, int mb, int mbx, int mby, int mbw, int b)
{
    return zs_ctx_f([&](int m) { return fl[m]; }, mb, mbx, mby, mbw, b);
}

template <class F>
__device__ __forceinline__ void zs_walk_mb(const ZwMbOut* M, const uint32_t* fl, int mb, int mbw, int t, F&& fn)
{
    const uint32_t f = fl[mb];
    if (f & ZS_SKIP) return;
    const int mbx = mb % mbw, mby = mb / mbw;
    const bool i4 = (f & ZS_I4) != 0;
    if (t == 1 && !i4) zs_walk(M->levels[16], zs_eob(M->levels[16]), 1, 0, zs_ctx(fl, mb, mbx, mby, mbw, 16), fn);
    if (t == (i4 ? 3 : 0))
        for (int b = 0; b < 16; b++)
            zs_walk(M->levels[b], zs_eob(M->levels[b]), t, i4 ? 0 : 1, zs_ctx(fl, mb, mbx, mby, mbw, b), fn);
    if (t == 2)
        for (int b = 17; b < 25; b++)
            zs_walk(M->levels[b], zs_eob(M->levels[b]), 2, 0, zs_ctx(fl, mb, mbx, mby, mbw, b), fn);
}

__device__ __forceinline__ void zs_rec(uint32_t& s, int bit)
{
    if (s >= 0xfffe0000u) s = ((s + 1) >> 1) & 0x7fff7fffu;
    s += 0x00010000u + (bit ? 1u : 0u);
}

extern "C" __global__ __launch_bounds__(256) void k_stats_flags(const ZwMbOut* __restrict__ mbs, int nmb,
                                                              uint32_t* __restrict__ fl)
{
    const int b = threadIdx.x & 31, f = blockIdx.y;
    const int mb = blockIdx.x * 8 + (threadIdx.x >> 5);
    const bool in = mb < nmb;
    const ZwMbOut& M = mbs[(size_t)f * nmb + (in ? mb : 0)];
    const bool i4 = M.luma_mode == 4;
    int nzb = 0;
    if (in && b < 25) {
        const int e = zs_eob(M.levels[b]);
        nzb = b < 16 ? e > (i4 ? 0 : 1) : (b == 16 ? (!i4 && e > 0) : e > 0);
    }
    const unsigned long long bal = __ballot(nzb);
    uint32_t m = (uint32_t)(bal >> (threadIdx.x & 32));
    if (m == 0) m = ZS_SKIP;
    if (in && b == 0) fl[(size_t)f * nmb + mb] = m | (i4 ? ZS_I4 : 0u);
}

#define ZS_FL_MAX (ZS_STRIPE + 1024)
extern "C" __global__ __launch_bounds__(ZS_HWG) void k_stats_hist(const ZwMbOut* __restrict__ mbs,
                                                                const uint32_t* __restrict__ flags, int mbw, int mbh,
                                                                uint2* __restrict__ part)
{
    extern __shared__ __attribute__((aligned(16))) uint8_t smem[];
    uint32_t* cp = (uint32_t*)smem;
    uint32_t* sfl = cp + ZS_COPIES * ZS_NCTR;
    const int st = blockIdx.x, f = blockIdx.y, tid = threadIdx.x, nst = gridDim.x;
    const int nmb = mbw * mbh;
    const ZwMbOut* F = mbs + (size_t)f * nmb;
    const uint32_t* fl = flags + (size_t)f * nmb;
    const int mb0 = st * ZS_STRIPE, mb1 = min(nmb, mb0 + ZS_STRIPE);
    const int lo = max(0, mb0 - min(mbw, 1024));
    for (int i = tid; i < ZS_COPIES * ZS_NCTR; i += ZS_HWG) cp[i] = 0;
    for (int m = lo + tid; m < mb1; m += ZS_HWG) sfl[m - lo] = fl[m];
    __syncthreads();
    auto flag = [&](int m) -> uint32_t { return m >= lo ? sfl[m - lo] : fl[m]; };
    uint32_t* my = cp + (tid & (ZS_COPIES - 1)) * ZS_NCTR;
    const int nit = (mb1 - mb0) * 25;
    struct Lv {
        uint32_t w[8];
    };
    auto lv_of = [&](int it) {
        Lv r;
        const uint32_t* p = (const uint32_t*)F[mb0 + it / 25].levels[it % 25];
#pragma unroll
        for (int k = 0; k < 8; k++) r.w[k] = p[k];
        return r;
    };
    Lv nx;
    if (tid < nit) nx = lv_of(tid);
    for (int it = tid; it < nit; it += ZS_HWG) {
        const Lv cur = nx;
        if (it + ZS_HWG < nit) nx = lv_of(it + ZS_HWG);
        const int mb = mb0 + it / 25, b = it % 25;
        const uint32_t fm = sfl[mb - lo];
        if (fm & ZS_SKIP) continue;
        const bool i4 = (fm & ZS_I4) != 0;
        if (b == 16 && i4) continue;
        const int t = b < 16 ? (i4 ? 3 : 0) : (b == 16 ? 1 : 2);
        const int first = b < 16 && !i4 ? 1 : 0;
        const int ctx = zs_ctx_f(flag, mb, mb % mbw, mb / mbw, mbw, b);
        int16_t lv[16];
#pragma unroll
        for (int k = 0; k < 8; k++) {
            lv[2 * k] = (int16_t)(cur.w[k] & 0xffffu);
            lv[2 * k + 1] = (int16_t)(cur.w[k] >> 16);
        }
        zs_walk(lv, zs_eob(lv), t, first, ctx, [&](int c, int bit) { atomicAdd(&my[c], 0x10000u + (bit ? 1u : 0u)); });
    }
    __syncthreads();
    for (int c = tid; c < ZS_NCTR; c += ZS_HWG) {
        uint32_t n = 0, o = 0;
#pragma unroll 8
        for (int j = 0; j < ZS_COPIES; j++) {
            const uint32_t v = cp[j * ZS_NCTR + c];
            n += v >> 16;
            o += v & 0xffffu;
        }
        part[((size_t)f * nst + st) * ZS_NCTR + c] = make_uint2(n, o);
    }
}

extern "C" __global__ __launch_bounds__(ZS_WG) void k_stats_final(const ZwMbOut* __restrict__ mbs,
                                                                 const uint32_t* __restrict__ flags, int mbw, int mbh,
                                                                 const uint2* __restrict__ part, int nst, int fl_lds,
                                                                 StatsOut* __restrict__ out)
{
    extern __shared__ __attribute__((aligned(16))) uint8_t smem[];
    int* heavy = (int*)smem;
    int* nheavy = heavy + ZS_NCTR;
    uint32_t* fll = (uint32_t*)(nheavy + 2);
    const int f = blockIdx.x, tid = threadIdx.x;
    const int nmb = mbw * mbh;
    const ZwMbOut* F = mbs + (size_t)f * nmb;
    const uint2* P = part + (size_t)f * nst * ZS_NCTR;
    if (tid < 2) nheavy[tid] = 0;
    __syncthreads();
    int nz = 0;
    for (int mb = tid; mb < nmb; mb += ZS_WG) {
        const uint32_t m = flags[(size_t)f * nmb + mb];
        if (fl_lds) fll[mb] = m;
        nz += (m & ZS_SKIP) ? 0 : 1;
    }
    if (nz) atomicAdd(&nheavy[1], nz);
    const uint32_t* fl = fl_lds ? fll : flags + (size_t)f * nmb;
    for (int c = tid; c < ZS_NCTR; c += ZS_WG) {
        uint32_t n = 0, o = 0;
        for (int st = 0; st < nst; st++) {
            const uint2 v = P[st * ZS_NCTR + c];
            n += v.x;
            o += v.y;
        }
        if (n <= 0xfffeu) {
            out[f].s[c] = (n << 16) | o;
        } else {
            const int k = atomicAdd(&nheavy[0], 1);
            heavy[k] = c;
        }
    }
    __syncthreads();
    const int wv = tid >> 6, lane = tid & 63, nh = nheavy[0];
    for (int k = wv; k < nh; k += ZS_WG / 64) {
        const int c = heavy[k], ct = c / (8 * 3 * 11);
        uint32_t s = 0;
        for (int st = 0; st < nst; st++) {
            const uint2 v = P[st * ZS_NCTR + c];
            if ((s >> 16) + v.x <= 0xfffeu) {
                s += (v.x << 16) + v.y;
                continue;
            }
            const int mb1 = min(nmb, (st + 1) * ZS_STRIPE);
            for (int base = st * ZS_STRIPE; base < mb1; base += 64) {
                const int mb = base + lane;
                uint32_t t = 0, o = 0;
                if (mb < mb1)
                    zs_walk_mb(F + mb, fl, mb, mbw, ct, [&](int cc, int bit) {
                        if (cc == c) {
                            t++;
                            o += bit ? 1u : 0u;
                        }
                    });
                uint32_t tsum = t;
#pragma unroll
                for (int o2 = 32; o2 >= 1; o2 >>= 1) tsum += __shfl_xor(tsum, o2);
                if ((s >> 16) + tsum <= 0xfffeu) {
                    uint32_t osum = o;
#pragma unroll
                    for (int o2 = 32; o2 >= 1; o2 >>= 1) osum += __shfl_xor(osum, o2);
                    s += (tsum << 16) + osum;
                } else {
                    for (int i = 0; i < 64 && base + i < mb1; i++) {
                        const uint32_t ti = (uint32_t)__shfl((int)t, i), oi = (uint32_t)__shfl((int)o, i);
                        if ((s >> 16) + ti <= 0xfffeu) {
                            s += (ti << 16) + oi;
                        } else {
                            uint32_t sl = s;
                            if (lane == 0)
                                zs_walk_mb(F + base + i, fl, base + i, mbw, ct, [&](int cc, int bit) {
                                    if (cc == c) zs_rec(sl, bit);
                                });
                            s = (uint32_t)__shfl((int)sl, 0);
                        }
                    }
                }
            }
        }
        if (lane == 0) out[f].s[c] = s;
    }
    if (tid == 0) {
        out[f].nonzero_mbs = (uint32_t)nheavy[1];
        out[f].total_mbs = (uint32_t)nmb;
    }
}

static int zs_stripes(int nmb) { return (nmb + ZS_STRIPE - 1) / ZS_STRIPE; }

static size_t zs_flag_bytes(int nmb) { return ((size_t)nmb * 4 + 7) & ~(size_t)7; }
extern "C" size_t zw_stats_scratch_bytes(int nmb, int nframes)
{
    return (size_t)nframes * (zs_flag_bytes(nmb) + (size_t)zs_stripes(nmb) * ZS_NCTR * sizeof(uint2));
}

extern "C" hipError_t zwk_stats(hipStream_t s, const ZwMbOut* mbs, int mbw, int mbh, void* scratch, void* out,
                                int nframes)
{
    static const bool attr = []() {
        (void)hipFuncSetAttribute((const void*)k_stats_hist, hipFuncAttributeMaxDynamicSharedMemorySize, 160 * 1024);
        (void)hipFuncSetAttribute((const void*)k_stats_final, hipFuncAttributeMaxDynamicSharedMemorySize,
                                  160 * 1024);
        return true;
    }();
    (void)attr;
    const int nmb = mbw * mbh, nst = zs_stripes(nmb);
    if (nmb <= 0 || nframes <= 0) return hipErrorInvalidValue;
    uint32_t* fl = (uint32_t*)scratch;
    uint2* part = (uint2*)((uint8_t*)scratch + (size_t)nframes * zs_flag_bytes(nmb));
    hipLaunchKernelGGL(k_stats_flags, dim3((nmb + 7) / 8, nframes), dim3(256), 0, s, mbs, nmb, fl);
    hipLaunchKernelGGL(k_stats_hist, dim3(nst, nframes), dim3(ZS_HWG), (size_t)(ZS_COPIES * ZS_NCTR + ZS_FL_MAX) * 4, s,
                       mbs, fl, mbw, mbh, part);
    const size_t lds0 = ZS_NCTR * 4 + 8;
    const int fl_lds = lds0 + (size_t)nmb * 4 <= 160 * 1024;
    hipLaunchKernelGGL(k_stats_final, dim3(nframes), dim3(ZS_WG), lds0 + (fl_lds ? (size_t)nmb * 4 : 0), s, mbs, fl,
                       mbw, mbh, part, nst, fl_lds, (StatsOut*)out);
    return hipGetLastError();
}
```

image-webp_amd/zwebp/__init__.py:

```python
import ctypes
import os
import threading
import weakref

import numpy as np

__all__ = [
    "ColorType", "EncoderParams", "WebPEncoder", "ZwError", "EncodingError", "DecodingError", "Context",
    "Frame", "Pipeline", "encode_frame_lossy", "encode_batch", "vp8_decode_frame", "decode_batch",
    "rgb_to_yuv420", "loop_filter_frame", "quant_blocks", "transform_quant_blocks", "library_path", "load_library",
    "UpsamplingMethod", "WebPDecoder", "decode_rgb", "decode_rgba", "vp8_decode_rgb", "decode_rgb_batch",
    "decode_rgb_batch_into", "decode_rgba_into", "decode_rgb_into",
    "decode_batch_device", "decode_batch_device_ptr", "decode_webp_batch_device",
    "decode_batch_device_resized", "decode_batch_device_resized_ptr", "decode_webp_batch_device_resized",
    "vp8_frame_dims",
    "encode_batch_device", "encode_batch_device_ptr", "encode_webp_batch_device",
    "yuv_to_rgb", "webp_parse", "encode_frame_lossless", "encode_alpha",
]

_HERE = os.path.dirname(os.path.abspath(__file__))
LIB_NAME = "libzwebp.so"


class ColorType:
# ... 83 lines not shown
class _Rect(ctypes.Structure):
    _fields_ = [("x", ctypes.c_uint32), ("y", ctypes.c_uint32), ("w", ctypes.c_uint32), ("h", ctypes.c_uint32)]


_VP, _SZ, _U32, _I, _U8 = ctypes.c_void_p, ctypes.c_size_t, ctypes.c_uint32, ctypes.c_int, ctypes.c_uint8
SIGNATURES = [
    ("zw_ctx_create", _I, [_I, ctypes.POINTER(_VP)]),
    ("zw_ctx_destroy", None, [_VP]),
    ("zw_ctx_release_buffers", None, [_VP]),
    ("zw_strerror", ctypes.c_char_p, [_I]),
    ("zw_bytes_free", None, [ctypes.POINTER(_Bytes)]),
    ("zw_frame_free", None, [ctypes.POINTER(_Frame)]),
    ("zw_encode_frame_lossy", _I, [_VP, _VP, _SZ, _U32, _U32, _I, _U8, _U8, ctypes.POINTER(_Bytes)]),
    ("zw_encode_frame_lossy_ex", _I, [_VP, _VP, _SZ, _U32, _U32, _I, _U8, _U8, _I, ctypes.POINTER(_Bytes)]),
    ("zw_encode_webp", _I, [_VP, _VP, _SZ, _U32, _U32, _I, _U8, _U8, ctypes.POINTER(_Bytes)]),
    ("zw_encode_webp_ex", _I, [_VP, _VP, _SZ, _U32, _U32, _I, ctypes.POINTER(_EncParams), ctypes.POINTER(_Metadata),
                               ctypes.POINTER(_Bytes)]),
    ("zw_encode_frame_lossless", _I, [_VP, _SZ, _U32, _U32, _I, _I, ctypes.POINTER(_Bytes)]),
    ("zw_encode_alpha", _I, [_VP, _SZ, _U32, _U32, _I, ctypes.POINTER(_Bytes)]),
    ("zw_encode_batch", _I, [_VP, _I, ctypes.POINTER(_Image), _U8, _U8, ctypes.POINTER(_Bytes)]),
    ("zw_encode_batch_ex", _I, [_VP, _I, ctypes.POINTER(_Image), _U8, _U8, _I, ctypes.POINTER(_Bytes)]),
    ("zw_encode_webp_batch", _I, [_VP, _I, ctypes.POINTER(_Image), _U8, _U8, ctypes.POINTER(_Bytes)]),
    ("zw_vp8_decode_frame", _I, [_VP, _VP, _SZ, ctypes.POINTER(_Frame)]),
    ("zw_vp8_decode_batch", _I, [_VP, _I, ctypes.POINTER(_VP), ctypes.POINTER(_SZ), ctypes.POINTER(_Frame)]),
    ("zw_vp8_decode_rgb", _I, [_VP, _VP, _SZ, _I, _I, ctypes.POINTER(_Bytes), ctypes.POINTER(_U32),
                               ctypes.POINTER(_U32)]),
    ("zw_vp8_decode_rgb_batch", _I, [_VP, _I, ctypes.POINTER(_VP), ctypes.POINTER(_SZ), _I, _I,
                                     ctypes.POINTER(_Bytes), _VP, _VP]),
    ("zw_vp8_decode_rgb_batch_into", _I, [_VP, _I, ctypes.POINTER(_VP), ctypes.POINTER(_SZ), _I, _I,
                                          ctypes.POINTER(_VP), ctypes.POINTER(_SZ), _U32, _VP, _VP]),
    ("zw_vp8_decode_batch_device", _I, [_VP, _I, ctypes.POINTER(_VP), ctypes.POINTER(_SZ),
                                        ctypes.POINTER(_DeviceImages), ctypes.POINTER(_U32), ctypes.POINTER(_U32)]),
    ("zw_vp8_decode_batch_device_resized", _I, [_VP, _I, ctypes.POINTER(_VP), ctypes.POINTER(_SZ),
                                                ctypes.POINTER(_DeviceImages), _U32, _U32, ctypes.POINTER(_Rect),
                                                ctypes.POINTER(_U32), ctypes.POINTER(_U32)]),
    ("zw_dbg_resize_taps", _I, [_U32, _U32, _U32, ctypes.POINTER(ctypes.c_int32)]),
    ("zw_vp8_decode_batch_device_resized_ex", _I, [_VP, _I, ctypes.POINTER(_VP), ctypes.POINTER(_SZ),
                                                   ctypes.POINTER(_DeviceImages), _U32, _U32, ctypes.POINTER(_Rect),
                                                   ctypes.POINTER(_U32), ctypes.POINTER(_U32), _I]),
    ("zw_dbg_resize_aa_taps", _I, [_U32, _U32, _U32, ctypes.POINTER(ctypes.c_int32), ctypes.POINTER(ctypes.c_int32),
                                   ctypes.POINTER(ctypes.c_uint16), _I]),
    ("zw_encode_batch_device", _I, [_VP, _I, ctypes.POINTER(_DeviceImages), _U32, _U32, _U8, _U8, _I,
                                    ctypes.POINTER(_Bytes)]),
    ("zw_pipe_set_input_device", _I, [_VP, ctypes.POINTER(_DeviceImages)]),
    ("zw_webp_parse", _I, [_VP, _SZ, ctypes.POINTER(_WebpInfo)]),
    ("zw_webp_decode_into", _I, [_VP, _VP, _SZ, _I, _I, _VP, _SZ, _U32, ctypes.POINTER(_U32),
                                 ctypes.POINTER(_U32)]),
    ("zw_webp_decode", _I, [_VP, _VP, _SZ, _I, _I, ctypes.POINTER(_Bytes), ctypes.POINTER(_U32),
                            ctypes.POINTER(_U32)]),
    ("zw_decode_rgb_kernel_ms", _I, [_VP, ctypes.POINTER(ctypes.c_float)]),
    ("zw_yuv_to_rgb", _I, [_VP, _VP, _VP, _VP, _U32, _U32, _U32, _U32, _I, _I, _VP]),
    ("zw_rgb_to_yuv420", _I, [_VP, _VP, _U32, _U32, _I, _VP, _VP, _VP]),
    ("zw_transform_quant_blocks", _I, [_VP, _SZ, _VP, _VP, _I, _I, _I, _I, _VP, _VP]),
    ("zw_transform_quant_blocks_device", _I, [_VP, _VP, _SZ, _VP, _VP, _I, _I, _I, _I, _VP, _VP]),
    ("zw_transform_quant_mbs", _I, [_VP, _I, _U32, _U32, _VP, _VP, _VP, _VP, _VP, _VP, _VP, _VP, _VP]),
    ("zw_xmb_seg_table_bytes", _SZ, [_I]),
    ("zw_xmb_seg_table", _I, [_I, _VP, _VP]),
    ("zw_transform_quant_mbs_device", _I, [_VP, _VP, _I, _U32, _U32, _VP, _VP, _VP, _VP, _VP, _VP, _VP, _VP, _VP]),
    ("zw_transform_quant_mbs_rgb", _I, [_VP, _I, _U32, _U32, _I, _VP, _VP, _VP, _VP, _VP, _VP, _VP]),
    ("zw_transform_quant_mbs_rgb_device", _I, [_VP, _VP, _I, _U32, _U32, _I, _VP, _SZ, _VP, _VP, _VP, _VP, _VP, _VP]),
    ("zw_quant_blocks", _I, [_VP, _I, _VP, _VP, _I, _I, _I, _U32, _I, _I, _I, _VP, _VP, _VP]),
    ("zw_loop_filter_frame", _I, [_VP, _VP, _VP, _VP, _U32, _U32, _VP, _I, _I, _I, _I, _I, _VP, _I, _I, _I]),
    ("zw_pipe_create", _I, [_VP, _I, _U32, _U32, _I, _U8, _U8, ctypes.POINTER(_VP)]),
    ("zw_pipe_destroy", None, [_VP]),
    ("zw_pipe_input_device_ptr", _VP, [_VP]),
    ("zw_pipe_upload", _I, [_VP, _I, _VP, _SZ]),
    ("zw_pipe_set_container", _I, [_VP, _I, ctypes.POINTER(_VP)]),
    ("zw_pipe_set_token_partitions", _I, [_VP, _I]),
    ("zw_decode_kernel_times", _I, [_VP, _VP]),
    ("zw_decode_stage_times", _I, [_VP, _VP]),
    ("zw_decode_token_ms", _I, [_VP, _VP]),
    ("zw_decode_token_stages", _I, [_VP, _VP]),
    ("zw_dbg_tokl_frame", _I, [_VP, _SZ, ctypes.POINTER(_I)]),
    ("zw_dbg_seam_stats", _I, [_VP, _I]),
    ("zw_pipe_encode", _I, [_VP]),
    ("zw_pipe_encode_repeat", _I, [_VP, _I]),
    ("zw_pipe_encode_host", _I, [_VP, _I, _VP]),
    ("zw_pipe_run_pass1", _I, [_VP, _I]),
    ("zw_pipe_run_device", _I, [_VP]),
    ("zw_pipe_output", _I, [_VP, _I, ctypes.POINTER(_Bytes)]),
    ("zw_pipe_read_planes", _I, [_VP, _I, _I, _VP, _VP, _VP]),
    ("zw_pipe_read_mbinfo", _I, [_VP, _I, _I, _VP, _VP]),
    ("zw_pipe_read_alpha", _I, [_VP, _I, _VP]),
    ("zw_pipe_enable_debug", _I, [_VP]),
    ("zw_pipe_read_debug", _I, [_VP, _I, _VP]),
    ("zw_pipe_read_segments", _I, [_VP, _I, _VP]),
    ("zw_pipe_read_probs", _I, [_VP, _I, _VP, ctypes.POINTER(_I)]),
    ("zw_pipe_kernel_times", _I, [_VP, ctypes.POINTER(ctypes.c_float), _I]),
    ("zw_pipe_lanes", _I, [_VP]),
    ("zw_pipe_launch_frames", _I, [_VP]),
    ("zw_host_threads", _I, []),
    ("zw_webp_parse_ex", _I, [_VP, _SZ, _I, ctypes.POINTER(_WebpInfoEx)]),
    ("zw_webp_decode_batch_device", _I, [_VP, _I, ctypes.POINTER(_VP), ctypes.POINTER(_SZ), _I,
                                         ctypes.POINTER(_DeviceImages), ctypes.POINTER(_U32), ctypes.POINTER(_U32)]),
    ("zw_webp_decode_ex", _I, [_VP, _VP, _SZ, _I, _I, _I, ctypes.POINTER(_Bytes), ctypes.POINTER(_U32),
                               ctypes.POINTER(_U32)]),
    ("zw_alph_decode", _I, [_VP, _VP, _SZ, _U32, _U32, _VP]),
    ("zw_dbg_alph_plane", _I, [_VP, _SZ, _U32, _U32, _VP, ctypes.POINTER(_I)]),
    ("zw_dbg_vp8l_decode", _I, [_VP, _SZ, _VP, ctypes.POINTER(_U32), ctypes.POINTER(_U32)]),
    ("zw_decode_alpha_times", _I, [_VP, ctypes.POINTER(ctypes.c_float)]),
]

_LIB = None


def load_library():
    global _LIB
    if _LIB is None:
        path = library_path()
        if not os.path.exists(path):
            raise ImportError(f"zwebp: HIP library not built ({path}); run `make -C image-webp_amd`")
        L = ctypes.CDLL(path)
        for name, res, args in SIGNATURES:
            fn = getattr(L, name)
            fn.restype = res
            fn.argtypes = args
        _LIB = L
    return _LIB


def _ptr(a):
    return ctypes.c_void_p(a.ctypes.data) if a is not None else None


def _check(rc, what, cls=ZwError):
    if rc != 0:
        raise cls(rc, what)


def host_threads():
    return load_library().zw_host_threads()


class Context:

    def __init__(self, device=0):
        L = load_library()
        h = ctypes.c_void_p()
        _check(L.zw_ctx_create(device, ctypes.byref(h)), "zw_ctx_create")
        self._h = h
        self._lib = L
        self.device = device

    @property
    def handle(self):
        return self._h

    def release_buffers(self):
        if self._h:
            self._lib.zw_ctx_release_buffers(self._h)

    def close(self):
        if self._h:
            self._lib.zw_ctx_destroy(self._h)
            self._h = None

    def __del__(self):
        try:
            self.close()
        except Exception:
            pass


_DEFAULT = {}


# ... 899 lines not shown
        self._h = h
        self.n, self.width, self.height, self.color = nframes, width, height, color
        self.mbw, self.mbh = (width + 15) // 16, (height + 15) // 16

    @property
    def input_ptr(self):
        return self._lib.zw_pipe_input_device_ptr(self._h)

    def upload(self, i, img):
        a = _as_u8(img)
        _check(self._lib.zw_pipe_upload(self._h, i, _ptr(a), a.size), "zw_pipe_upload")

    def set_container(self, host_frames=None, enable=True):
        self._host_frames = [_as_u8(f) for f in host_frames] if host_frames is not None else None
        ptrs = None
        if self._host_frames is not None:
            ptrs = (ctypes.c_void_p * len(self._host_frames))(*[f.ctypes.data for f in self._host_frames])
        _check(self._lib.zw_pipe_set_container(self._h, 1 if enable else 0, ptrs), "zw_pipe_set_container",
               EncodingError)

    def set_input(self, tensor, layout="chw", scale=None, bias=None):
        if tensor is None:
            _check(self._lib.zw_pipe_set_input_device(self._h, None), "zw_pipe_set_input_device", EncodingError)
            self._input = None
            return
        import torch
        d, n, w, h, _ = _tensor_images(tensor, layout, scale, bias, self.ctx.device)
        if (n, w, h) != (self.n, self.width, self.height):
            raise ValueError(f"the tensor must hold {self.n} frames of {self.width}x{self.height}")
        torch.cuda.current_stream(torch.device("cuda", self.ctx.device)).synchronize()
        _check(self._lib.zw_pipe_set_input_device(self._h, ctypes.byref(d)), "zw_pipe_set_input_device",
               EncodingError)
        self._input = tensor

    def set_token_partitions(self, n):
        _check(self._lib.zw_pipe_set_token_partitions(self._h, n), "zw_pipe_set_token_partitions", EncodingError)

    def encode(self):
        _check(self._lib.zw_pipe_encode(self._h), "zw_pipe_encode", EncodingError)

    def encode_repeat(self, n):
        _check(self._lib.zw_pipe_encode_repeat(self._h, int(n)), "zw_pipe_encode_repeat", EncodingError)

    def encode_host(self, batches):
        nb = len(batches)
        arrs = [_as_u8(im) for bt in batches for im in bt]
        if nb == 0 or len(arrs) != nb * self.n:
            raise ValueError("nb batches of n frames")
        want = self.width * self.height * (1, 2, 3, 4)[self.color]
        if any(a.size != want for a in arrs):
            raise ValueError("every frame must be width*height*bpp bytes")
        ptrs = (ctypes.c_void_p * len(arrs))(*[a.ctypes.data for a in arrs])
        _check(self._lib.zw_pipe_encode_host(self._h, nb, ptrs), "zw_pipe_encode_host", EncodingError)

    def run_pass1(self, write_recon=True):
        _check(self._lib.zw_pipe_run_pass1(self._h, 1 if write_recon else 0), "zw_pipe_run_pass1", EncodingError)

    def run_device(self):
        _check(self._lib.zw_pipe_run_device(self._h), "zw_pipe_run_device", EncodingError)

    def output(self, i):
        b = _Bytes()
        _check(self._lib.zw_pipe_output(self._h, i, ctypes.byref(b)), "zw_pipe_output")
        return _take_bytes(self._lib, b)

    def planes(self, i, which=0):
        ys, cs = self.mbw * self.mbh * 256, self.mbw * self.mbh * 64
        y, u, v = np.zeros(ys, np.uint8), np.zeros(cs, np.uint8), np.zeros(cs, np.uint8)
        _check(self._lib.zw_pipe_read_planes(self._h, i, which, _ptr(y), _ptr(u), _ptr(v)), "zw_pipe_read_planes")
        return y, u, v

    def mbinfo(self, i, pass_=2):
        nmb = self.mbw * self.mbh
        modes = np.zeros((nmb, 20), np.uint8)
        levels = np.zeros((nmb, 25, 16), np.int16)
        _check(self._lib.zw_pipe_read_mbinfo(self._h, i, pass_, _ptr(modes), _ptr(levels)), "zw_pipe_read_mbinfo")
        return modes, levels

    def alpha(self, i):
        a = np.zeros(self.mbw * self.mbh, np.uint8)
        _check(self._lib.zw_pipe_read_alpha(self._h, i, _ptr(a)), "zw_pipe_read_alpha")
        return a

    def enable_debug(self):
        _check(self._lib.zw_pipe_enable_debug(self._h), "zw_pipe_enable_debug")

    def i4_dump(self, i):
        d = np.zeros(self.mbw * self.mbh * 16 * 34, np.int32)
        _check(self._lib.zw_pipe_read_debug(self._h, i, _ptr(d)), "zw_pipe_read_debug")
        return d.reshape(self.mbw * self.mbh, 16, 34)

    def segments(self, i):
        q = np.zeros(4, np.int32)
        _check(self._lib.zw_pipe_read_segments(self._h, i, _ptr(q)), "read_segments")
        return q

    def probs(self, i):
        pr = np.zeros(4 * 8 * 3 * 11, np.uint8)
        sp = ctypes.c_int()
        _check(self._lib.zw_pipe_read_probs(self._h, i, _ptr(pr), ctypes.byref(sp)), "zw_pipe_read_probs")
        return pr, sp.value

    @property
    def lanes(self):
        return self._lib.zw_pipe_lanes(self._h)

    @property
    def launch_frames(self):
        return self._lib.zw_pipe_launch_frames(self._h)

    def kernel_times(self):
        ms = (ctypes.c_float * 9)()
        n = self._lib.zw_pipe_kernel_times(self._h, ms, 9)
        _check(n, "zw_pipe_kernel_times")
        return list(ms)

    def close(self):
        if self._h:
            self._lib.zw_pipe_destroy(self._h)
            self._h = None

    def __del__(self):
        try:
            self.close()
        except Exception:
            pass
```

include/zwebp.h:

```cpp
#ifndef ZWEBP_H
#define ZWEBP_H
#include <stddef.h>
#include <stdint.h>

#ifdef __cplusplus
extern "C" {
#endif

enum {
    ZW_OK = 0,
    ZW_EINVALID_DIMENSIONS = 1,
    ZW_EINVALID_BUFFER_SIZE = 2,
    ZW_EINVAL = 3,
    ZW_EDEVICE = 4,
    ZW_EUNSUPPORTED = 5,
    ZW_ENOMEM = 6,
    ZW_EVP8_MAGIC = 10,
    ZW_ECOLORSPACE = 11,
    ZW_ELUMA_MODE = 12,
    ZW_EINTRA_MODE = 13,
    ZW_ECHROMA_MODE = 14,
    ZW_EBITSTREAM = 15,
    ZW_EUNSUPPORTED_FEATURE = 16,
    ZW_ENOT_ENOUGH_INIT_DATA = 17,
// ... 118 lines not shown
                          int cap);
int zw_encode_batch_device(zw_ctx *ctx, int n, const zw_device_images *in, uint32_t width, uint32_t height,
                           uint8_t quality, uint8_t method, int token_partitions, zw_bytes *outs);
int zw_webp_parse(const uint8_t *data, size_t len, zw_webp_info *info);
int zw_webp_decode(zw_ctx *ctx, const uint8_t *data, size_t len, int bpp, int upsampling, zw_bytes *out,
                   uint32_t *width, uint32_t *height);
int zw_webp_decode_into(zw_ctx *ctx, const uint8_t *data, size_t len, int bpp, int upsampling, uint8_t *out,
                        size_t out_len, uint32_t stride_bytes, uint32_t *width, uint32_t *height);
enum { ZW_WEBP_ALPHA = 1 };
typedef struct {
    uint32_t width, height;
    int has_alpha, is_lossy, is_lossless, is_animated;
    uint64_t vp8_offset, vp8_len;
    uint64_t alph_offset, alph_len;
} zw_webp_info_ex;
int zw_webp_parse_ex(const uint8_t *data, size_t len, int flags, zw_webp_info_ex *info);
int zw_webp_decode_batch_device(zw_ctx *ctx, int n, const uint8_t *const *files, const size_t *lens, int flags,
                                const zw_device_images *out, uint32_t *width, uint32_t *height);
int zw_webp_decode_ex(zw_ctx *ctx, const uint8_t *data, size_t len, int bpp, int upsampling, int flags, zw_bytes *out,
                      uint32_t *width, uint32_t *height);
int zw_alph_decode(zw_ctx *ctx, const uint8_t *payload, size_t len, uint32_t width, uint32_t height,
                   uint8_t *plane_out);
int zw_dbg_alph_plane(const uint8_t *payload, size_t len, uint32_t width, uint32_t height, uint8_t *plane,
                      int *filter);
int zw_dbg_vp8l_decode(const uint8_t *data, size_t len, uint32_t *argb_out, uint32_t *width, uint32_t *height);
int zw_decode_alpha_times(zw_ctx *ctx, float *ms);
int zw_decode_kernel_times(zw_ctx *ctx, float *ms);
int zw_decode_stage_times(zw_ctx *ctx, float *ms);
int zw_decode_token_ms(zw_ctx *ctx, float *ms);
int zw_decode_token_stages(zw_ctx *ctx, float *ms);
int zw_dbg_tokl_frame(const uint8_t *vp8, size_t len, int *match);
int zw_dbg_seam_stats(uint64_t *out, int reset);
int zw_decode_rgb_kernel_ms(zw_ctx *ctx, float *ms);

int zw_rgb_to_yuv420(zw_ctx *ctx, const uint8_t *img, uint32_t width, uint32_t height, int bpp, uint8_t *y,
                     uint8_t *u, uint8_t *v);
int zw_yuv_to_rgb(zw_ctx *ctx, const uint8_t *y, const uint8_t *u, const uint8_t *v, uint32_t width,
                  uint32_t height, uint32_t y_stride, uint32_t uv_stride, int bpp, int upsampling, uint8_t *out);
int zw_quant_blocks(zw_ctx *ctx, int n, const int32_t *coeffs, const uint8_t *ctx0, int ctype, int first,
                    int use_trellis, uint32_t lambda, int q_dc, int q_ac, int matrix_type, const uint8_t *probs,
                    int32_t *levels, int32_t *dequant);
int zw_transform_quant_blocks(zw_ctx *ctx, size_t n, const uint8_t *src, const uint8_t *pred, int q_dc, int q_ac,
                              int matrix_type, int first, int16_t *levels, uint8_t *recon);
int zw_transform_quant_blocks_device(zw_ctx *ctx, void *stream, size_t n, const void *d_src, const void *d_pred,
                                     int q_dc, int q_ac, int matrix_type, int first, void *d_levels, void *d_recon);
#define ZW_XMB_RECORD_BYTES 96
int zw_transform_quant_mbs(zw_ctx *ctx, int nframes, uint32_t mbw, uint32_t mbh, const uint8_t *y, const uint8_t *u,
                           const uint8_t *v, const uint8_t *recs, const int32_t *seg_qi, int16_t *levels, uint8_t *ry,
                           uint8_t *ru, uint8_t *rv);
size_t zw_xmb_seg_table_bytes(int nframes);
int zw_xmb_seg_table(int nframes, const int32_t *seg_qi, void *out);
int zw_transform_quant_mbs_device(zw_ctx *ctx, void *stream, int nframes, uint32_t mbw, uint32_t mbh, const void *d_y,
                                  const void *d_u, const void *d_v, const void *d_recs, const void *d_segs,
                                  void *d_levels, void *d_ry, void *d_ru, void *d_rv);
int zw_transform_quant_mbs_rgb(zw_ctx *ctx, int nframes, uint32_t width, uint32_t height, int bpp, const uint8_t *img,
                               const uint8_t *recs, const int32_t *seg_qi, int16_t *levels, uint8_t *ry, uint8_t *ru,
                               uint8_t *rv);
int zw_transform_quant_mbs_rgb_device(zw_ctx *ctx, void *stream, int nframes, uint32_t width, uint32_t height, int bpp,
                                      const void *d_img, size_t img_stride, const void *d_recs, const void *d_segs,
                                      void *d_levels, void *d_ry, void *d_ru, void *d_rv);
int zw_loop_filter_frame(zw_ctx *ctx, uint8_t *y, uint8_t *u, uint8_t *v, uint32_t mbw, uint32_t mbh,
                         const uint8_t *mb_flags, int filter_type, int filter_level, int sharpness,
                         int segments_enabled, int seg_delta_values, const int8_t seg_lf_level[4],
                         int lf_adj_enabled, int ref_delta0, int mode_delta0);

typedef struct zw_pipe zw_pipe;
int zw_pipe_create(zw_ctx *ctx, int nframes, uint32_t width, uint32_t height, int color, uint8_t quality,
                   uint8_t method, zw_pipe **out);
void zw_pipe_destroy(zw_pipe *p);
void *zw_pipe_input_device_ptr(zw_pipe *p);
int zw_pipe_upload(zw_pipe *p, int frame, const uint8_t *data, size_t len);
int zw_pipe_set_container(zw_pipe *p, int enable, const uint8_t *const *host_frames);
int zw_pipe_set_input_device(zw_pipe *p, const zw_device_images *in);
int zw_pipe_set_token_partitions(zw_pipe *p, int nparts);
int zw_pipe_encode(zw_pipe *p);
int zw_pipe_encode_repeat(zw_pipe *p, int n);
int zw_pipe_encode_host(zw_pipe *p, int nb, const uint8_t *const *frames);
int zw_pipe_run_device(zw_pipe *p);
int zw_pipe_output(zw_pipe *p, int frame, zw_bytes *out);
int zw_pipe_run_pass1(zw_pipe *p, int write_recon);
int zw_pipe_read_planes(zw_pipe *p, int frame, int which , uint8_t *y, uint8_t *u, uint8_t *v);
int zw_pipe_read_mbinfo(zw_pipe *p, int frame, int pass, uint8_t *modes , int16_t *levels );
int zw_pipe_read_alpha(zw_pipe *p, int frame, uint8_t *alpha);
int zw_pipe_enable_debug(zw_pipe *p);
int zw_pipe_read_debug(zw_pipe *p, int frame, int32_t *out);
int zw_pipe_read_segments(zw_pipe *p, int frame, int32_t *seg_qi);
int zw_pipe_read_probs(zw_pipe *p, int frame, uint8_t *probs, int *skip_prob);
int zw_pipe_lanes(zw_pipe *p);
int zw_pipe_launch_frames(zw_pipe *p);
int zw_pipe_kernel_times(zw_pipe *p, float *ms, int n);
int zw_host_threads(void);

#ifdef __cplusplus
}
#endif
#endif
```

Before: 4639 encodes/s.

## Emit stats flags and EOBs from encode kernels; compact stats and pack writer

Pass 1 now writes per-macroblock nonzero flags for luma and chroma directly from LDS, so the stats stage can skip the separate flag-scan kernel that re-reads all level records. The stats histogram builds a compacted list of full blocks and counts the all-zero classes with ballots, so only nonzero blocks have their levels reloaded. Pass 2 writes per-block EOBs alongside the sizes, and a new half-wave-per-macroblock pack writer uses those EOBs with a prefix scan. Debug entry points are added for verification. The cost is extra global writes in the encode kernels and more complex stats and pack kernels.

```diff
diff --git a/image-webp_amd/csrc/zw_enc_kernels.hip b/image-webp_amd/csrc/zw_enc_kernels.hip
--- a/image-webp_amd/csrc/zw_enc_kernels.hip
+++ b/image-webp_amd/csrc/zw_enc_kernels.hip
@@ -52,6 +52,9 @@
     int* dbg;
     uint8_t* rows;
     uint32_t* sizes;
+    uint8_t* eobs;
+    uint32_t* fl_luma;
+    uint8_t* fl_chroma;
     int nframes;
 };
 
@@ -1859,6 +1862,18 @@
     uint32_t* dst = (uint32_t*)&o->levels[first_blk][0];
     const uint32_t* srcl = (const uint32_t*)&C.M->lev[first_blk][0];
     for (int k = C.lane; k < nblk * 8; k += 64) dst[k] = zero ? 0u : srcl[k];
+}
+
+DI void chroma_flags(const Ctx& C, int first_blk, int nq, uint8_t* dst)
+{
+    const int lane = C.lane;
+    const uint32_t v = lane < nq * 32 ? ((const uint32_t*)&C.M->lev[first_blk][0])[lane] : 0u;
+    const unsigned long long bal = __ballot(v != 0);
+    if (lane < nq) {
+        const uint32_t h = (uint32_t)(bal >> (32 * lane));
+        dst[lane] = (uint8_t)(((h & 0xffu) != 0) | ((h & 0xff00u) != 0) << 1 | ((h & 0xff0000u) != 0) << 2 |
+                              ((h >> 24) != 0) << 3);
+    }
 }
 
 struct UvQ {
@@ -2526,6 +2541,7 @@
                     e = (v >> 16) ? 2 * q + 2 : ((v & 0xffffu) ? 2 * q + 1 : e);
                 }
             }
+            if (lane < 25) a.eobs[((size_t)C.f * nmb + (size_t)C.mby * mbw + C.mbx) * 25 + lane] = (uint8_t)e;
             const int r16 = red16(e);
             const int es = __builtin_amdgcn_readlane(r16, 0) + __builtin_amdgcn_readlane(r16, 16);
             if (lane == 0)
@@ -2534,6 +2550,18 @@
     } else {
         write_levels(C, 0, 17, false);
         if (lane == 0) o->skip = 0;
+        if (a.fl_luma) {
+            uint32_t any = 0;
+            if (lane < 17) {
+                const uint32_t* lw = (const uint32_t*)C.M->lev[lane];
+                any = lm != 4 && lane < 16 ? lw[0] >> 16 : lw[0];
+#pragma unroll
+                for (int q = 1; q < 8; q++) any |= lw[q];
+                if (lm == 4 && lane == 16) any = 0;
+            }
+            const uint32_t m = (uint32_t)__ballot(any != 0) | (lm == 4 ? 1u << 25 : 0u);
+            if (lane == 0) a.fl_luma[(size_t)C.f * nmb + (size_t)C.mby * mbw + C.mbx] = m;
+        }
     }
     if (lane == 0) {
         o->luma_mode = (uint8_t)lm;
@@ -2605,6 +2633,8 @@
             ZwMbOut* o = a.out + (size_t)f * nmb + (size_t)mby * mbw + mbx;
             if (pl == 0 && lane == 0) o->chroma_mode = (uint8_t)cm;
             write_levels(C, 17 + 4 * pl, 4, false);
+            if (a.fl_chroma)
+                chroma_flags(C, 17 + 4 * pl, 1, a.fl_chroma + ((size_t)f * nmb + (size_t)mby * mbw + mbx) * 2 + pl);
             wsync();
         }
     }
@@ -2651,6 +2681,7 @@
             ZwMbOut* o = a.out + (size_t)F.f * nmb + (size_t)mby * mbw + mbx;
             if (lane == 0) o->chroma_mode = (uint8_t)cm;
             write_levels(C, 17, 8, false);
+            if (a.fl_chroma) chroma_flags(C, 17, 2, a.fl_chroma + ((size_t)F.f * nmb + (size_t)mby * mbw + mbx) * 2);
             wsync();
         }
     }
@@ -3040,11 +3071,15 @@
 extern "C" hipError_t zwk_encode(hipStream_t s, int pass, const uint8_t* Y, const uint8_t* U, const uint8_t* V,
                                  const uint8_t* alpha, const ZwFrameParams* params, const ZwLevelCosts* lcost,
                                  int8_t* derr, ZwMbOut* out, uint8_t* ry, uint8_t* ru, uint8_t* rv, size_t ysz,
-                                 size_t csz, int mbw, int mbh, int nframes, int* dbg, uint8_t* rows, uint32_t* sizes)
+                                 size_t csz, int mbw, int mbh, int nframes, int* dbg, uint8_t* rows, uint32_t* sizes,
+                                 uint8_t* eobs, uint32_t* fl_luma, uint8_t* fl_chroma)
 {
     EncArgs a;
+    a.fl_luma = pass == 1 && fl_chroma ? fl_luma : nullptr;
+    a.fl_chroma = a.fl_luma ? fl_chroma : nullptr;
     a.dbg = dbg;
-    a.sizes = pass == 2 ? sizes : nullptr;
+    a.sizes = pass == 2 && eobs ? sizes : nullptr;
+    a.eobs = eobs;
     a.Y = Y; a.U = U; a.V = V; a.alpha = alpha; a.params = params; a.lcost = lcost; a.derr = derr; a.out = out;
     a.ry = ry; a.ru = ru; a.rv = rv; a.ysz = ysz; a.csz = csz; a.mbw = mbw; a.mbh = mbh; a.pass = pass;
     a.rows = rows;
diff --git a/image-webp_amd/csrc/zw_host.cpp b/image-webp_amd/csrc/zw_host.cpp
--- a/image-webp_amd/csrc/zw_host.cpp
+++ b/image-webp_amd/csrc/zw_host.cpp
@@ -36,10 +36,16 @@
                         size_t ysz, size_t csz, uint8_t* alpha, uint32_t* histo, int nframes);
 hipError_t zwk_segments(hipStream_t s, uint32_t* histo, const ZwFrameParams* tmpl, ZwFrameParams* params,
                         int nframes);
-hipError_t zwk_stats(hipStream_t s, const ZwMbOut* mbs, int mbw, int mbh, void* scratch, void* out, int nframes);
+hipError_t zwk_stats(hipStream_t s, const ZwMbOut* mbs, int mbw, int mbh, void* scratch, void* out, int nframes,
+                     const uint32_t* fl_luma, const uint8_t* fl_chroma);
+hipError_t zwk_stats_flags(hipStream_t s, const ZwMbOut* mbs, int nmb, int nframes, const uint32_t* fl_luma,
+                           const uint8_t* fl_chroma, uint32_t* fl);
 size_t zw_stats_scratch_bytes(int nmb, int nframes);
 hipError_t zwk_pack(hipStream_t s, const ZwMbOut* mbs, int nmb, int nframes, uint8_t* eobs, uint32_t* sizes,
-                     unsigned long long* counter, unsigned long long* frame_info, uint8_t* out, int sizes_ready);
+                     unsigned long long* counter, unsigned long long* frame_info, uint8_t* out, int sizes_ready,
+                     int writer = -1);
+hipError_t zwk_pack_write(hipStream_t s, const ZwMbOut* mbs, int nmb, int nframes, const uint8_t* eobs,
+                          const uint32_t* offs, const unsigned long long* frame_info, uint8_t* out, int writer);
 hipError_t zwk_fdct_quant(hipStream_t s, const void* src, const void* pred, size_t n, const ZwMatrix* m, int first,
                           void* levels, void* recon, int cus);
 hipError_t zwk_xform_mb(hipStream_t s, const uint8_t* Y, const uint8_t* U, const uint8_t* V, int src_bpp, int w,
@@ -54,7 +60,8 @@
 hipError_t zwk_encode(hipStream_t s, int pass, const uint8_t* Y, const uint8_t* U, const uint8_t* V,
                       const uint8_t* alpha, const ZwFrameParams* params, const ZwLevelCosts* lcost, int8_t* derr,
                       ZwMbOut* out, uint8_t* ry, uint8_t* ru, uint8_t* rv, size_t ysz, size_t csz, int mbw, int mbh,
-                      int nframes, int* dbg, uint8_t* rows, uint32_t* sizes = nullptr);
+                      int nframes, int* dbg, uint8_t* rows, uint32_t* sizes = nullptr, uint8_t* eobs = nullptr,
+                      uint32_t* fl_luma = nullptr, uint8_t* fl_chroma = nullptr);
 size_t zwk_encode_rows_bytes(int mbw, int mbh, int nframes);
 int zwk_encode_max_mbw(int rows);
 int zwk_encode_fp(int pass, int mbw, int nframes);
@@ -497,6 +504,8 @@
     int* d_dbg = nullptr;
     ZwStatsOut* d_stats = nullptr;
     void* d_stats_tmp = nullptr;
+    uint32_t* d_fl_luma = nullptr;
+    uint8_t* d_fl_chroma = nullptr;
     bool host_stats = false;
     uint8_t* d_eobs = nullptr;
     uint32_t* d_sizes = nullptr;
@@ -640,8 +649,16 @@
               hipMalloc(&p->d_pack2, N * p->pack_stride) == hipSuccess;
     ok = ok && hipMemset(p->d_histo, 0, N * 256 * sizeof(uint32_t)) == hipSuccess;
     p->host_stats = getenv("ZW_HOST_STATS") != nullptr;
+    const size_t stats_scr = zw_stats_scratch_bytes(p->nmb, n);
     ok = ok && (p->host_stats || (hipMalloc(&p->d_stats, N * sizeof(ZwStatsOut)) == hipSuccess &&
-                                  hipMalloc(&p->d_stats_tmp, zw_stats_scratch_bytes(p->nmb, n)) == hipSuccess));
+                                  hipMalloc(&p->d_stats_tmp, stats_scr + N * p->nmb * 6) == hipSuccess));
+    {
+        const char* e = getenv("ZW_STATS_PASS_FLAGS");
+        if (ok && !p->host_stats && !(e && *e && atoi(e) == 0)) {
+            p->d_fl_luma = (uint32_t*)((uint8_t*)p->d_stats_tmp + stats_scr);
+            p->d_fl_chroma = (uint8_t*)(p->d_fl_luma + N * p->nmb);
+        }
+    }
     const int G = pipe_lanes_for(n, ctx->device, p->mbw);
     p->lanes.resize(G);
     for (int g = 0; ok && g < G; g++) {
@@ -820,7 +837,8 @@
                      p->d_params + F, nullptr, p->d_derr + F * p->mbw * 4, p->d_out1 + F * p->nmb,
                      write_recon ? p->d_ry + F * p->ysz : nullptr, write_recon ? p->d_ru + F * p->csz : nullptr,
                      write_recon ? p->d_rv + F * p->csz : nullptr, p->ysz, p->csz, p->mbw, p->mbh, na, nullptr,
-                     L.d_rows));
+                     L.d_rows, nullptr, nullptr, p->d_fl_luma ? p->d_fl_luma + F * p->nmb : nullptr,
+                     p->d_fl_luma ? p->d_fl_chroma + F * p->nmb * 2 : nullptr));
     if (timed) HIPOK(hipEventRecord(L.ev[EV_P1_END], s));
     return ZW_OK;
 }
@@ -938,7 +956,8 @@
                      p->d_params + F, p->d_lcost + F, p->d_derr + F * p->mbw * 4, p->d_out2 + F * p->nmb,
                      p->d_ry + F * p->ysz, p->d_ru + F * p->csz, p->d_rv + F * p->csz, p->ysz, p->csz, p->mbw, p->mbh,
                      na, p->d_dbg ? p->d_dbg + F * p->nmb * 16 * 34 : nullptr, L.d_rows,
-                     pass2_sizes(p) ? p->d_sizes + F * p->nmb : nullptr));
+                     pass2_sizes(p) ? p->d_sizes + F * p->nmb : nullptr,
+                     pass2_sizes(p) ? p->d_eobs + F * p->nmb * 25 : nullptr));
     if (timed) HIPOK(hipEventRecord(L.ev[EV_P2_END], s));
     return ZW_OK;
 }
@@ -1174,7 +1193,8 @@
                 const size_t F = (size_t)first(k);
                 HIPOK(zwk_stats(L.stream, p->d_out1 + F * p->nmb, p->mbw, p->mbh,
                                 (uint8_t*)p->d_stats_tmp + zw_stats_scratch_bytes(p->nmb, (int)F), p->d_stats + F,
-                                count(k)));
+                                count(k), p->d_fl_luma ? p->d_fl_luma + F * p->nmb : nullptr,
+                                p->d_fl_luma ? p->d_fl_chroma + F * p->nmb * 2 : nullptr));
             }
             if (!r) HIPOK(hipEventRecord(L.pass_done(k, 1), L.stream));
         }
@@ -1564,6 +1584,60 @@
         if (levels) memcpy(levels + (size_t)i * 400, tmp[i].levels, 800);
     }
     return ZW_OK;
+}
+
+extern "C" int zw_pipe_read_stats_flags(zw_pipe* p, int frame, int from_records, uint32_t* flags)
+{
+    if (!p || frame < 0 || frame >= p->n || !flags) return ZW_EINVAL;
+    if (!from_records && !p->d_fl_luma) return ZW_EUNSUPPORTED;
+    HIPOK(hipSetDevice(p->ctx->device));
+    const size_t F = (size_t)frame;
+    uint32_t* d = nullptr;
+    if (hipMalloc(&d, (size_t)p->nmb * 4) != hipSuccess) return ZW_ENOMEM;
+    hipError_t e = zwk_stats_flags(nullptr, p->d_out1 + F * p->nmb, p->nmb, 1,
+                                   from_records ? nullptr : p->d_fl_luma + F * p->nmb,
+                                   from_records ? nullptr : p->d_fl_chroma + F * p->nmb * 2, d);
+    if (e == hipSuccess) e = hipMemcpy(flags, d, (size_t)p->nmb * 4, hipMemcpyDeviceToHost);
+    (void)hipFree(d);
+    return e == hipSuccess ? ZW_OK : ZW_EDEVICE;
+}
+
+extern "C" int zw_pipe_debug_pack(zw_pipe* p, int frame, int mode, uint8_t* eobs, uint8_t* stream, size_t cap,
+                                  size_t* bytes)
+{
+    if (!p || frame < 0 || frame >= p->n || mode < 0 || mode > 2 || !eobs || !stream || !bytes) return ZW_EINVAL;
+    HIPOK(hipSetDevice(p->ctx->device));
+    const size_t F = (size_t)frame, nmb = (size_t)p->nmb;
+    const ZwMbOut* recs = p->d_out2 + F * nmb;
+    uint8_t *d_eobs = nullptr, *d_out = nullptr;
+    uint32_t* d_sizes = nullptr;
+    unsigned long long* d_ctr = nullptr;
+    unsigned long long info[2] = {0, 0};
+    hipError_t e = hipMalloc(&d_eobs, nmb * 25);
+    if (e == hipSuccess) e = hipMalloc(&d_out, p->pack_stride);
+    if (e == hipSuccess) e = hipMalloc(&d_sizes, nmb * 4);
+    if (e == hipSuccess) e = hipMalloc(&d_ctr, (ZW_PACK_CTR_WORDS + 2) * sizeof(unsigned long long));
+    if (e == hipSuccess) e = hipMemset(d_ctr, 0, (ZW_PACK_CTR_WORDS + 2) * sizeof(unsigned long long));
+    if (e == hipSuccess)
+        e = zwk_pack(nullptr, recs, p->nmb, 1, d_eobs, d_sizes, d_ctr, d_ctr + ZW_PACK_CTR_WORDS, d_out, 0,
+                     mode == 1 ? 1 : 0);
+    if (e == hipSuccess && mode == 0) {
+        e = hipMemcpy(d_eobs, p->d_eobs + F * nmb * 25, nmb * 25, hipMemcpyDeviceToDevice);
+        if (e == hipSuccess) e = hipMemset(d_out, 0, p->pack_stride);
+        if (e == hipSuccess)
+            e = zwk_pack_write(nullptr, recs, p->nmb, 1, d_eobs, d_sizes, d_ctr + ZW_PACK_CTR_WORDS, d_out, 0);
+    }
+    if (e == hipSuccess) e = hipMemcpy(info, d_ctr + ZW_PACK_CTR_WORDS, sizeof info, hipMemcpyDeviceToHost);
+    if (e == hipSuccess) e = hipMemcpy(eobs, d_eobs, nmb * 25, hipMemcpyDeviceToHost);
+    int r = e == hipSuccess ? ZW_OK : ZW_EDEVICE;
+    if (!r && (info[0] != 0 || info[1] > cap)) r = ZW_EINVAL;
+    if (!r && hipMemcpy(stream, d_out, info[1], hipMemcpyDeviceToHost) != hipSuccess) r = ZW_EDEVICE;
+    if (!r) *bytes = (size_t)info[1];
+    (void)hipFree(d_eobs);
+    (void)hipFree(d_out);
+    (void)hipFree(d_sizes);
+    (void)hipFree(d_ctr);
+    return r;
 }
 
 extern "C" int zw_pipe_read_probs(zw_pipe* p, int frame, uint8_t* probs, int* skip_prob)
diff --git a/image-webp_amd/csrc/zw_pack_kernels.hip b/image-webp_amd/csrc/zw_pack_kernels.hip
--- a/image-webp_amd/csrc/zw_pack_kernels.hip
+++ b/image-webp_amd/csrc/zw_pack_kernels.hip
@@ -1,4 +1,5 @@
 #include "zw_dev.h"
+#include <cstdlib>
 
 #ifndef PK_WAVES
 #define PK_WAVES 4
@@ -89,7 +90,7 @@
     }
 }
 
-extern "C" __global__ __launch_bounds__(64 * PK_WAVES) void k_pack_write(
+extern "C" __global__ __launch_bounds__(64 * PK_WAVES) void k_pack_write_dense(
     const ZwMbOut* __restrict__ mbs, int nmb, int nframes, const uint8_t* __restrict__ eobs,
     const uint32_t* __restrict__ offs, const unsigned long long* __restrict__ frame_info, uint8_t* __restrict__ out)
 {
@@ -142,16 +143,72 @@
     }
 }
 
+#define PK_HALF 2
+extern "C" __global__ __launch_bounds__(64 * PK_WAVES) void k_pack_write(
+    const ZwMbOut* __restrict__ mbs, int nmb, int nframes, const uint8_t* __restrict__ eobs,
+    const uint32_t* __restrict__ offs, const unsigned long long* __restrict__ frame_info, uint8_t* __restrict__ out)
+{
+    const size_t total = (size_t)nmb * nframes;
+    const size_t mb0 = ((size_t)blockIdx.x * PK_WAVES + (threadIdx.x >> 6)) * PK_HALF + ((threadIdx.x >> 5) & 1);
+    const bool in = mb0 < total;
+    const size_t mb = in ? mb0 : 0;
+    const int b = threadIdx.x & 31;
+    const ZwMbOut& M = mbs[mb];
+    const int eob = b < 25 ? (int)eobs[mb * 25 + b] : 0;
+    const uint32_t hw = *(const uint32_t*)&M;
+    const uint32_t bp = b < 8 ? *(const uint16_t*)&M.bpred[2 * b] : 0u;
+    uint8_t* o = out + frame_info[2 * (mb / nmb)] + offs[mb];
+    uint32_t w[8];
+    const uint32_t* W = (const uint32_t*)&M.levels[min(b, 24)][0];
+#pragma unroll
+    for (int q = 0; q < 8; q++) w[q] = 2 * q < eob ? W[q] : 0u;
+    const int luma = (int)(hw & 255u), chroma = (int)((hw >> 8) & 255u), skip = (int)((hw >> 16) & 255u),
+              seg = (int)(hw >> 24);
+    const int hdr = 1 + (luma == 4 ? 8 : 0);
+    int pre = eob;
+#pragma unroll
+    for (int d = 1; d < 32; d <<= 1) {
+        const int v = __shfl_up(pre, d, 32);
+        if (b >= d) pre += v;
+    }
+    pre -= eob;
+    if (!in) return;
+    if (b == 0) o[0] = (uint8_t)(luma | (skip << 3) | (seg << 4) | (chroma << 6));
+    if (luma == 4 && b < 8) o[1 + b] = (uint8_t)((bp & 15u) | (((bp >> 8) & 15u) << 4));
+    if (b < 25) o[hdr + b] = (uint8_t)eob;
+    int16_t* lv = (int16_t*)(o + hdr + 25) + pre;
+#pragma unroll
+    for (int q = 0; q < 8; q++) {
+        if (2 * q < eob) lv[2 * q] = (int16_t)(w[q] & 0xffffu);
+        if (2 * q + 1 < eob) lv[2 * q + 1] = (int16_t)(w[q] >> 16);
+    }
+}
+
+extern "C" hipError_t zwk_pack_write(hipStream_t s, const ZwMbOut* mbs, int nmb, int nframes, const uint8_t* eobs,
+                                     const uint32_t* offs, const unsigned long long* frame_info, uint8_t* out,
+                                     int writer)
+{
+    static const int dense = [] { const char* e = getenv("ZW_PACK_DENSE"); return e && *e ? atoi(e) : 0; }();
+    const size_t total = (size_t)nmb * nframes;
+    if (writer < 0 ? dense : writer) {
+        hipLaunchKernelGGL(k_pack_write_dense, dim3((unsigned)((total + PK_WAVES - 1) / PK_WAVES)), dim3(64 * PK_WAVES),
+                           0, s, mbs, nmb, nframes, eobs, offs, frame_info, out);
+    } else {
+        constexpr size_t per = PK_WAVES * PK_HALF;
+        hipLaunchKernelGGL(k_pack_write, dim3((unsigned)((total + per - 1) / per)), dim3(64 * PK_WAVES), 0, s, mbs, nmb,
+                           nframes, eobs, offs, frame_info, out);
+    }
+    return hipGetLastError();
+}
+
 extern "C" hipError_t zwk_pack(hipStream_t s, const ZwMbOut* mbs, int nmb, int nframes, uint8_t* eobs, uint32_t* sizes,
                                unsigned long long* counter, unsigned long long* frame_info, uint8_t* out,
-                               int sizes_ready)
+                               int sizes_ready, int writer)
 {
     const size_t total = (size_t)nmb * nframes;
     const unsigned grid = (unsigned)((total + PK_WAVES - 1) / PK_WAVES);
     if (!sizes_ready)
         hipLaunchKernelGGL(k_pack_size, dim3(grid), dim3(64 * PK_WAVES), 0, s, mbs, nmb, nframes, eobs, sizes);
     hipLaunchKernelGGL(k_pack_scan, dim3(nframes), dim3(1024), 0, s, sizes, nmb, counter, frame_info);
-    hipLaunchKernelGGL(k_pack_write, dim3(grid), dim3(64 * PK_WAVES), 0, s, mbs, nmb, nframes, eobs, sizes, frame_info,
-                       out);
-    return hipGetLastError();
-}
+    return zwk_pack_write(s, mbs, nmb, nframes, eobs, sizes, frame_info, out, writer);
+}
diff --git a/image-webp_amd/csrc/zw_stats_kernels.hip b/image-webp_amd/csrc/zw_stats_kernels.hip
--- a/image-webp_amd/csrc/zw_stats_kernels.hip
+++ b/image-webp_amd/csrc/zw_stats_kernels.hip
@@ -144,6 +144,12 @@
     s += 0x00010000u + (bit ? 1u : 0u);
 }
 
+__device__ __forceinline__ uint32_t zs_combine(uint32_t luma, uint32_t uv)
+{
+    const uint32_t m = (luma & 0x1ffffu) | ((uv & 0xfu) << 17) | (((uv >> 8) & 0xfu) << 21);
+    return (m ? m : ZS_SKIP) | (luma & ZS_I4);
+}
+
 extern "C" __global__ __launch_bounds__(256) void k_stats_flags(const ZwMbOut* __restrict__ mbs, int nmb,
                                                               uint32_t* __restrict__ fl)
 {
@@ -164,48 +170,99 @@
 }
 
 #define ZS_FL_MAX (ZS_STRIPE + 1024)
+#define ZS_HIST_LDS ((size_t)(ZS_COPIES * ZS_NCTR + ZS_FL_MAX + 1) * 4 + (size_t)ZS_STRIPE * 25 * 2)
+static_assert(ZS_STRIPE * 25 <= 4096, "a list entry keeps the item in 12 bits");
+static_assert(ZS_HWG % 64 == 0, "whole waves");
 extern "C" __global__ __launch_bounds__(ZS_HWG) void k_stats_hist(const ZwMbOut* __restrict__ mbs,
-                                                                const uint32_t* __restrict__ flags, int mbw, int mbh,
+                                                                uint32_t* flags, const uint32_t* __restrict__ fl_luma,
+                                                                const uint8_t* __restrict__ fl_chroma, int mbw, int mbh,
                                                                 uint2* __restrict__ part)
 {
     extern __shared__ __attribute__((aligned(16))) uint8_t smem[];
     uint32_t* cp = (uint32_t*)smem;
     uint32_t* sfl = cp + ZS_COPIES * ZS_NCTR;
+    int* nlist = (int*)(sfl + ZS_FL_MAX);
+    uint16_t* list = (uint16_t*)(nlist + 1);
     const int st = blockIdx.x, f = blockIdx.y, tid = threadIdx.x, nst = gridDim.x;
     const int nmb = mbw * mbh;
     const ZwMbOut* F = mbs + (size_t)f * nmb;
-    const uint32_t* fl = flags + (size_t)f * nmb;
+    uint32_t* fl = flags + (size_t)f * nmb;
+    const bool pf = fl_luma != nullptr;
+    const uint32_t* fll = fl_luma + (size_t)f * nmb;
+    const uint16_t* flc = (const uint16_t*)fl_chroma + (size_t)f * nmb;
+    auto gflag = [&](int m) -> uint32_t { return pf ? zs_combine(fll[m], flc[m]) : fl[m]; };
     const int mb0 = st * ZS_STRIPE, mb1 = min(nmb, mb0 + ZS_STRIPE);
     const int lo = max(0, mb0 - min(mbw, 1024));
     for (int i = tid; i < ZS_COPIES * ZS_NCTR; i += ZS_HWG) cp[i] = 0;
-    for (int m = lo + tid; m < mb1; m += ZS_HWG) sfl[m - lo] = fl[m];
+    if (tid == 0) *nlist = 0;
+    for (int m = lo + tid; m < mb1; m += ZS_HWG) {
+        const uint32_t v = gflag(m);
+        sfl[m - lo] = v;
+        if (pf && m >= mb0) fl[m] = v;
+    }
     __syncthreads();
-    auto flag = [&](int m) -> uint32_t { return m >= lo ? sfl[m - lo] : fl[m]; };
+    auto flag = [&](int m) -> uint32_t { return m >= lo ? sfl[m - lo] : gflag(m); };
     uint32_t* my = cp + (tid & (ZS_COPIES - 1)) * ZS_NCTR;
-    const int nit = (mb1 - mb0) * 25;
+    const int nit = (mb1 - mb0) * 25, lane = tid & 63;
+    uint32_t ne[12];
+#pragma unroll
+    for (int k = 0; k < 12; k++) ne[k] = 0;
+    for (int i0 = tid - lane; i0 < nit; i0 += ZS_HWG) {
+        const int it = i0 + lane;
+        int cls = -1, ctx = 0;
+        bool full = false;
+        if (it < nit) {
+            const int mb = mb0 + it / 25, b = it % 25;
+            const uint32_t fm = sfl[mb - lo];
+            const bool i4 = (fm & ZS_I4) != 0;
+            if (!(fm & ZS_SKIP) && !(b == 16 && i4)) {
+                ctx = zs_ctx_f(flag, mb, mb % mbw, mb / mbw, mbw, b);
+                full = ((fm >> b) & 1u) != 0;
+                if (!full) cls = (b < 16 ? (i4 ? 3 : 0) : (b == 16 ? 1 : 2)) * 3 + ctx;
+            }
+        }
+#pragma unroll
+        for (int k = 0; k < 12; k++) ne[k] += (uint32_t)__popcll(__ballot(cls == k));
+        const unsigned long long fb = __ballot(full);
+        if (fb) {
+            int base = 0;
+            if (lane == 0) base = atomicAdd(nlist, __popcll(fb));
+            base = __shfl(base, 0);
+            if (full) list[base + __popcll(fb & ((1ull << lane) - 1ull))] = (uint16_t)(it | (ctx << 12));
+        }
+    }
+    {
+        uint32_t mine = 0;
+#pragma unroll
+        for (int k = 0; k < 12; k++) mine = lane == k ? ne[k] : mine;
+        if (lane < 12 && mine) {
+            const int t = lane / 3;
+            atomicAdd(&my[((t * 8 + (t == 0 ? 1 : 0)) * 3 + lane % 3) * 11], mine << 16);
+        }
+    }
+    __syncthreads();
+    const int nl = *nlist;
     struct Lv {
         uint32_t w[8];
     };
-    auto lv_of = [&](int it) {
+    auto lv_of = [&](int i) {
         Lv r;
+        const int it = list[i] & 0xfff;
         const uint32_t* p = (const uint32_t*)F[mb0 + it / 25].levels[it % 25];
 #pragma unroll
         for (int k = 0; k < 8; k++) r.w[k] = p[k];
         return r;
     };
     Lv nx;
-    if (tid < nit) nx = lv_of(tid);
-    for (int it = tid; it < nit; it += ZS_HWG) {
+    if (tid < nl) nx = lv_of(tid);
+    for (int i = tid; i < nl; i += ZS_HWG) {
         const Lv cur = nx;
-        if (it + ZS_HWG < nit) nx = lv_of(it + ZS_HWG);
+        if (i + ZS_HWG < nl) nx = lv_of(i + ZS_HWG);
+        const int it = list[i] & 0xfff, ctx = list[i] >> 12;
         const int mb = mb0 + it / 25, b = it % 25;
-        const uint32_t fm = sfl[mb - lo];
-        if (fm & ZS_SKIP) continue;
-        const bool i4 = (fm & ZS_I4) != 0;
-        if (b == 16 && i4) continue;
+        const bool i4 = (sfl[mb - lo] & ZS_I4) != 0;
         const int t = b < 16 ? (i4 ? 3 : 0) : (b == 16 ? 1 : 2);
         const int first = b < 16 && !i4 ? 1 : 0;
-        const int ctx = zs_ctx_f(flag, mb, mb % mbw, mb / mbw, mbw, b);
         int16_t lv[16];
 #pragma unroll
         for (int k = 0; k < 8; k++) {
@@ -328,7 +385,7 @@
 }
 
 extern "C" hipError_t zwk_stats(hipStream_t s, const ZwMbOut* mbs, int mbw, int mbh, void* scratch, void* out,
-                                int nframes)
+                                int nframes, const uint32_t* fl_luma, const uint8_t* fl_chroma)
 {
     static const bool attr = []() {
         (void)hipFuncSetAttribute((const void*)k_stats_hist, hipFuncAttributeMaxDynamicSharedMemorySize, 160 * 1024);
@@ -341,12 +398,36 @@
     if (nmb <= 0 || nframes <= 0) return hipErrorInvalidValue;
     uint32_t* fl = (uint32_t*)scratch;
     uint2* part = (uint2*)((uint8_t*)scratch + (size_t)nframes * zs_flag_bytes(nmb));
-    hipLaunchKernelGGL(k_stats_flags, dim3((nmb + 7) / 8, nframes), dim3(256), 0, s, mbs, nmb, fl);
-    hipLaunchKernelGGL(k_stats_hist, dim3(nst, nframes), dim3(ZS_HWG), (size_t)(ZS_COPIES * ZS_NCTR + ZS_FL_MAX) * 4, s,
-                       mbs, fl, mbw, mbh, part);
+    if (!fl_luma || !fl_chroma) {
+        fl_luma = nullptr;
+        fl_chroma = nullptr;
+        hipLaunchKernelGGL(k_stats_flags, dim3((nmb + 7) / 8, nframes), dim3(256), 0, s, mbs, nmb, fl);
+    }
+    hipLaunchKernelGGL(k_stats_hist, dim3(nst, nframes), dim3(ZS_HWG), ZS_HIST_LDS, s, mbs, fl, fl_luma, fl_chroma, mbw,
+                       mbh, part);
     const size_t lds0 = ZS_NCTR * 4 + 8;
     const int fl_lds = lds0 + (size_t)nmb * 4 <= 160 * 1024;
-    hipLaunchKernelGGL(k_stats_final, dim3(nframes), dim3(ZS_WG), lds0 + (fl_lds ? (size_t)nmb * 4 : 0), s, mbs, fl,
-                       mbw, mbh, part, nst, fl_lds, (StatsOut*)out);
+    hipLaunchKernelGGL(k_stats_final, dim3(nframes), dim3(ZS_WG), lds0 + (fl_lds ? (size_t)nmb * 4 : 0), s, mbs,
+                       (const uint32_t*)fl, mbw, mbh, part, nst, fl_lds, (StatsOut*)out);
     return hipGetLastError();
 }
+
+extern "C" __global__ __launch_bounds__(256) void k_stats_combine(const uint32_t* __restrict__ fl_luma,
+                                                                const uint8_t* __restrict__ fl_chroma, size_t n,
+                                                                uint32_t* __restrict__ fl)
+{
+    const size_t i = (size_t)blockIdx.x * 256 + threadIdx.x;
+    if (i < n) fl[i] = zs_combine(fl_luma[i], ((const uint16_t*)fl_chroma)[i]);
+}
+extern "C" hipError_t zwk_stats_flags(hipStream_t s, const ZwMbOut* mbs, int nmb, int nframes, const uint32_t* fl_luma,
+                                      const uint8_t* fl_chroma, uint32_t* fl)
+{
+    if (nmb <= 0 || nframes <= 0) return hipErrorInvalidValue;
+    if (fl_luma && fl_chroma) {
+        const size_t n = (size_t)nmb * nframes;
+        hipLaunchKernelGGL(k_stats_combine, dim3((unsigned)((n + 255) / 256)), dim3(256), 0, s, fl_luma, fl_chroma, n, fl);
+    } else {
+        hipLaunchKernelGGL(k_stats_flags, dim3((nmb + 7) / 8, nframes), dim3(256), 0, s, mbs, nmb, fl);
+    }
+    return hipGetLastError();
+}
diff --git a/image-webp_amd/zwebp/__init__.py b/image-webp_amd/zwebp/__init__.py
--- a/image-webp_amd/zwebp/__init__.py
+++ b/image-webp_amd/zwebp/__init__.py
@@ -189,6 +189,8 @@
     ("zw_pipe_read_planes", _I, [_VP, _I, _I, _VP, _VP, _VP]),
     ("zw_pipe_read_mbinfo", _I, [_VP, _I, _I, _VP, _VP]),
     ("zw_pipe_read_alpha", _I, [_VP, _I, _VP]),
+    ("zw_pipe_read_stats_flags", _I, [_VP, _I, _I, _VP]),
+    ("zw_pipe_debug_pack", _I, [_VP, _I, _I, _VP, _VP, _SZ, ctypes.POINTER(_SZ)]),
     ("zw_pipe_enable_debug", _I, [_VP]),
     ("zw_pipe_read_debug", _I, [_VP, _I, _VP]),
     ("zw_pipe_read_segments", _I, [_VP, _I, _VP]),
@@ -1254,6 +1256,21 @@
         _check(self._lib.zw_pipe_read_alpha(self._h, i, _ptr(a)), "zw_pipe_read_alpha")
         return a
 
+    def stats_flags(self, i, from_records=False):
+        fl = np.zeros(self.mbw * self.mbh, np.uint32)
+        _check(self._lib.zw_pipe_read_stats_flags(self._h, i, 1 if from_records else 0, _ptr(fl)),
+               "zw_pipe_read_stats_flags")
+        return fl
+
+    def debug_pack(self, i, mode=0):
+        nmb = self.mbw * self.mbh
+        eobs = np.zeros((nmb, 25), np.uint8)
+        stream = np.zeros(nmb * 834, np.uint8)
+        n = _SZ(0)
+        _check(self._lib.zw_pipe_debug_pack(self._h, i, mode, _ptr(eobs), _ptr(stream), stream.size, ctypes.byref(n)),
+               "zw_pipe_debug_pack")
+        return eobs, stream[:n.value].copy()
+
     def enable_debug(self):
         _check(self._lib.zw_pipe_enable_debug(self._h), "zw_pipe_enable_debug")
 
diff --git a/include/zwebp.h b/include/zwebp.h
--- a/include/zwebp.h
+++ b/include/zwebp.h
@@ -224,6 +224,9 @@
 int zw_pipe_read_planes(zw_pipe *p, int frame, int which , uint8_t *y, uint8_t *u, uint8_t *v);
 int zw_pipe_read_mbinfo(zw_pipe *p, int frame, int pass, uint8_t *modes , int16_t *levels );
 int zw_pipe_read_alpha(zw_pipe *p, int frame, uint8_t *alpha);
+int zw_pipe_read_stats_flags(zw_pipe *p, int frame, int from_records, uint32_t *flags );
+int zw_pipe_debug_pack(zw_pipe *p, int frame, int mode, uint8_t *eobs , uint8_t *stream, size_t cap,
+                       size_t *bytes);
 int zw_pipe_enable_debug(zw_pipe *p);
 int zw_pipe_read_debug(zw_pipe *p, int frame, int32_t *out);
 int zw_pipe_read_segments(zw_pipe *p, int frame, int32_t *seg_qi);
```

Measured after the change: 4639 encodes/s, median of 3. No clear change (-0.0%).
